# felipeagc/sycl-ray-tracer

Measured on AMD Instinct MI355X. Metric: Mrays/s, higher is better.
Workload: dtype f32

## Files before the change

### include/rt_mi355x.h

```cpp
#ifndef RT_MI355X_H
#define RT_MI355X_H

#include <stddef.h>
#include <stdint.h>

#ifdef __cplusplus
extern "C" {
#endif

#define RT_ABI_VERSION 8

typedef enum rt_status {
    RT_OK = 0,
    RT_ERR_INVALID = -1,
    RT_ERR_NO_DEVICE = -2,
    RT_ERR_HIP = -3,
    RT_ERR_OOM = -4,
    RT_ERR_UNSUPPORTED = -5
} rt_status;

#define RT_TEX_SIZE 512u
#define RT_TEX_CHANNELS 4u
#define RT_TEX_MAX_LAYERS 128u

// ... 6 lines not shown
    int32_t height;
} rt_camera;

int rt_camera_init(rt_camera* out, int32_t width, int32_t height, const float center[3],
                   const float dir[3], float focal_length);

enum { RT_MAT_NONE = 0, RT_MAT_DIFFUSE = 1, RT_MAT_METALLIC = 2, RT_MAT_DIELECTRIC = 3 };
enum { RT_TEX_COLOR = 0, RT_TEX_IMAGE = 1 };

typedef struct rt_material {
    uint32_t type;
    uint32_t tex_kind;
    float color[3];
    uint32_t tex_layer;
    float emissive[3];
    float roughness;
    float ior;
} rt_material;

typedef struct rt_instance {
    float transform[16];
    float normal_mat[9];
    uint32_t material;
} rt_instance;

typedef struct rt_scene_desc {
    uint32_t n_vertices;
    const float* positions;
    const float* normals;
    const float* uvs;
    uint32_t n_triangles;
    const uint32_t* indices;
    const uint32_t* tri_instance;
    uint32_t n_instances;
    const rt_instance* instances;
    uint32_t n_materials;
    const rt_material* materials;
    uint32_t n_layers;
    const uint8_t* textures;
    float sky[3];
} rt_scene_desc;

typedef struct rt_scene rt_scene;
typedef struct rt_renderer rt_renderer;

enum { RT_BVH_DEFAULT = 0, RT_BVH_LBVH = 1, RT_BVH_SAH = 2, RT_BVH_LBVH_GPU = 3 };

int rt_scene_create(const rt_scene_desc* desc, int device, int bvh_kind, rt_scene** out);
void rt_scene_destroy(rt_scene* scene);

#define RT_SCENE_UPDATABLE 1u
int rt_scene_create_ex(const rt_scene_desc* desc, int device, int bvh_kind, uint32_t flags, rt_scene** out);
#define RT_SCENE_KEEP_PREVIOUS 2u

typedef struct rt_scene_update_desc {
    uint32_t n_instances;
    const rt_instance* instances;
    uint32_t n_vertices;
    const float* positions;
    const float* normals;
} rt_scene_update_desc;
typedef struct rt_update_stats { double device_ms; uint32_t launches; uint32_t refit_nodes; } rt_update_stats;
int rt_scene_update(rt_scene* scene, const rt_scene_update_desc* u, rt_update_stats* stats);

typedef struct rt_scene_info_t {
    uint32_t n_triangles;
    uint32_t n_nodes;
    uint32_t max_depth;
    uint32_t max_leaf_tris;
    float bounds_lo[3];
    float bounds_hi[3];
    double sah_cost;
    uint64_t device_bytes;
    uint32_t n_leaf_records;
    uint32_t n_split_triangles;
} rt_scene_info_t;
int rt_scene_info(const rt_scene* scene, rt_scene_info_t* out);

int rt_scene_check_bvh(const rt_scene* scene);
int rt_scene_count_visits(const rt_scene* scene, uint32_t n, const float* org, const float* dir, int mode,
                          uint64_t* node_visits, uint64_t* tri_tests, float* t, uint32_t* tri);

int rt_intersect_batch(rt_scene* scene, uint32_t n, const float* org, const float* dir, float* t,
                       float* u, float* v, uint32_t* tri);

enum { RT_QUERY_CLOSEST = 0, RT_QUERY_ANY = 1 };
#define RT_TRI_REJECTED 0xFFFFFFFEu
typedef struct rt_ray_query {
    uint32_t n;
    uint32_t mode;
    const float* org;
    const float* dir;
    const float* tmax;
    float* t;
    float* u;
    float* v;
    uint32_t* tri;
    uint8_t* occluded;
} rt_ray_query;
int rt_trace_rays(rt_scene* scene, const rt_ray_query* q);
int rt_trace_rays_device(rt_scene* scene, const rt_ray_query* q, void* stream);

typedef struct rt_path_query {
    uint32_t n;
    uint32_t max_depth;
    uint32_t samples;
    uint32_t rr_start;
    const float* org;
    const float* dir;
    const uint32_t* rng;
    uint32_t* rng_out;
    float* radiance;
    uint32_t* rays;
} rt_path_query;
int rt_trace_paths(rt_scene* scene, const rt_path_query* q);
int rt_trace_paths_device(rt_scene* scene, const rt_path_query* q, void* stream);

enum {
    RT_RENDERER_MEGAKERNEL = 0,
    RT_RENDERER_WAVEFRONT = 1
};
enum { RT_SEED_DEFAULT = 0, RT_SEED_WAVEFRONT = 1, RT_SEED_MEGAKERNEL = 2 };

int rt_renderer_create(int kind, rt_scene* scene, int32_t width, int32_t height,
                       uint32_t max_depth, uint32_t sample_count, uint32_t seed_mode,
                       rt_renderer** out);
void rt_renderer_destroy(rt_renderer* r);

int rt_renderer_set_tile(rt_renderer* r, uint32_t rank, uint32_t world, uint32_t strip_rows);
int32_t rt_renderer_local_rows(const rt_renderer* r);
int32_t rt_renderer_global_row(const rt_renderer* r, int32_t local_row);

int rt_renderer_set_profiling(rt_renderer* r, int enable);

int rt_renderer_set_russian_roulette(rt_renderer* r, uint32_t start_bounce);

int rt_renderer_set_frame_seed(rt_renderer* r, uint32_t salt);

#define RT_SCHED_ALL_BOUNCES 0xFFFFFFFFu
typedef struct rt_schedule {
    uint32_t finish_depth;
    uint32_t samples_per_launch;
    uint32_t stream_lanes;
    int32_t requeue;
    uint32_t reorder;
    uint32_t matsort;
    int32_t cost_order;
    uint32_t hip_graph;
    uint32_t fused_bounce;
    int32_t pixel_slices;
} rt_schedule;
int rt_renderer_set_schedule(rt_renderer* r, const rt_schedule* s);
int rt_renderer_get_schedule(const rt_renderer* r, rt_schedule* out);

enum {
    RT_K_MEGAKERNEL = 0,
    RT_K_WF_INIT = 1,
    RT_K_WF_GENERATE = 2,
    RT_K_WF_EXTEND = 3,
    RT_K_WF_SHADE = 4,
    RT_K_WF_SHADE_REORDER = 5,
    RT_K_WF_SHADE_MATSORT = 6,
    RT_K_WF_FINISH = 7,
    RT_K_WF_FINISH_REQUEUE = 8,
    RT_K_WF_TILE_ORDER = 9,
    RT_K_WF_RESOLVE = 10,
    RT_K_FILL_BLACK = 11,
    RT_K_WF_SHOOT = 12,
    RT_K_BLOCK_RESOLVE = 13,
    RT_K_COUNT = 16
};

typedef struct rt_stats {
    uint64_t rays;
    double seconds;
    double device_ms;
    double hot_kernel_ms;
    uint32_t hot_kernel_launches;
    uint32_t launches;
    uint32_t launches_by_kernel[RT_K_COUNT];
    uint32_t stream_lanes;
    uint32_t samples_per_launch;
    uint32_t finish_depth;
    uint32_t cost_ordered;
    double kernel_ms[RT_K_COUNT];
    uint32_t hw_queues;
    uint32_t pixel_slices;
} rt_stats;

int rt_render_frame(rt_renderer* r, const rt_camera* cam, float* rgba_f32, uint8_t* rgba_u8,
                    rt_stats* stats);

int rt_render_frame_device(rt_renderer* r, const rt_camera* cam, void* d_rgba_f32,
                           void* d_rgba_u8, void* stream, rt_stats* stats);

int rt_render_frame_begin(rt_renderer* r, const rt_camera* cam, void* d_rgba_f32, void* d_rgba_u8, void* stream);
int rt_render_frame_end(rt_renderer* r, rt_stats* stats);

int rt_renderer_set_progressive(rt_renderer* r, int enable);
int rt_render_frame_continue(rt_renderer* r, uint32_t samples, float* rgba_f32, uint8_t* rgba_u8, rt_stats* stats);
int rt_render_frame_continue_device(rt_renderer* r, uint32_t samples, void* d_rgba_f32, void* d_rgba_u8,
                                    void* stream, rt_stats* stats);
int rt_renderer_accumulated_samples(const rt_renderer* r, uint32_t* out);

int rt_renderer_block_grid(const rt_renderer* r, uint32_t* blocks_x, uint32_t* blocks_y);
int rt_render_frame_continue_blocks(rt_renderer* r, uint32_t samples, const uint32_t* blocks, uint32_t n_blocks,
                                    float* rgba_f32, uint8_t* rgba_u8, rt_stats* stats);
int rt_render_frame_continue_blocks_device(rt_renderer* r, uint32_t samples, const uint32_t* blocks, uint32_t n_blocks,
                                           void* d_rgba_f32, void* d_rgba_u8, void* stream, rt_stats* stats);
int rt_renderer_block_samples(const rt_renderer* r, uint32_t* out);
int rt_renderer_adapt(rt_renderer* r, float threshold, uint32_t min_samples, uint32_t* blocks_out, uint32_t* n_out);
int rt_render_frame_continue_adaptive(rt_renderer* r, uint32_t samples, float threshold, uint32_t min_samples,
                                      float* rgba_f32, uint8_t* rgba_u8, rt_stats* stats, uint32_t* n_blocks_out);
int rt_render_frame_continue_adaptive_device(rt_renderer* r, uint32_t samples, float threshold, uint32_t min_samples,
                                             void* d_rgba_f32, void* d_rgba_u8, void* stream, rt_stats* stats,
                                             uint32_t* n_blocks_out);
int rt_renderer_block_errors(const rt_renderer* r, float* out);

int rt_scene_gbuffer(rt_scene* scene, const rt_camera* cam, float* albedo, float* normal, float* position);
int rt_scene_gbuffer_device(rt_scene* scene, const rt_camera* cam, void* d_albedo, void* d_normal, void* d_position, void* stream);

int rt_scene_gbuffer_motion(rt_scene* scene, const rt_camera* cam, float* albedo, float* normal, float* position, float* prev_position);
// ... 93 lines not shown
```

### sycl-ray-tracer_amd/csrc/rt_abi.hip

```cpp
#include "bvh_quantise.h"
#include "rt_internal.h"

namespace rtlib {
thread_local std::string g_err;

int copy_out(const rt_renderer* r, int rc, float* rgba_f32, uint8_t* rgba_u8) {
    if (rc != RT_OK) return rc;
    if (rgba_f32 && r->n_local) HIPCHK(hipMemcpy(rgba_f32, r->d_f32, (size_t)r->n_local * 16, hipMemcpyDeviceToHost));
    if (rgba_u8 && r->n_local) HIPCHK(hipMemcpy(rgba_u8, r->d_u8, (size_t)r->n_local * 4, hipMemcpyDeviceToHost));
    return RT_OK;
}
}

extern "C" {

const char* rt_last_error(void) { return g_err.c_str(); }
int rt_abi_version(void) { return RT_ABI_VERSION; }

int rt_device_count(void) {
    int n = 0;
    hipError_t e = hipGetDeviceCount(&n);
    if (e != hipSuccess) return fail(RT_ERR_NO_DEVICE, std::string("hipGetDeviceCount: ") + hipGetErrorString(e));
    return n;
}

int rt_camera_init(rt_camera* out, int32_t width, int32_t height, const float center[3], const float dir_in[3],
                   float focal_length) {
    if (!out || !center || !dir_in || width <= 0 || height <= 0) return fail(RT_ERR_INVALID, "bad camera arguments");
    auto norm = [](const float v[3], float o[3]) {
        float inv = 1.0f / std::sqrt((v[0] * v[0] + v[1] * v[1]) + v[2] * v[2]);
        o[0] = v[0] * inv, o[1] = v[1] * inv, o[2] = v[2] * inv;
    };
    auto cross = [](const float a[3], const float b[3], float o[3]) {
        o[0] = a[1] * b[2] - a[2] * b[1], o[1] = a[2] * b[0] - a[0] * b[2], o[2] = a[0] * b[1] - a[1] * b[0];
    };
    float dir[3], right[3], up[3], tmp[3];
    const float world_up[3] = {0.0f, 1.0f, 0.0f};
    norm(dir_in, dir);
    cross(dir, world_up, tmp), norm(tmp, right);
    cross(right, dir, tmp), norm(tmp, up);
    const float vp0 = 1.0f * ((float)width / (float)height), vp1 = 1.0f;
    const float du_div = (float)width / (vp0 * 2.0f), dv_div = (float)height / (vp1 * 2.0f);
    for (int a = 0; a < 3; ++a) {
        const float viewport_u = (-right[a]) * vp0, viewport_v = up[a] * vp1;
        out->center[a] = center[a];
        out->pixel00[a] = ((center[a] + viewport_u) + viewport_v) + dir[a] * focal_length;
        out->delta_u[a] = right[a] / du_div;
        out->delta_v[a] = (-up[a]) / dv_div;
    }
    out->width = width, out->height = height;
    return RT_OK;
}

int rt_scene_create(const rt_scene_desc* desc, int device, int bvh_kind, rt_scene** out) { return rt_scene_create_ex(desc, device, bvh_kind, 0u, out); }

int rt_scene_create_ex(const rt_scene_desc* desc, int device, int bvh_kind, uint32_t flags, rt_scene** out) {
    if (!out) return fail(RT_ERR_INVALID, "null output pointer");
    *out = nullptr;
    if (flags & ~(RT_SCENE_UPDATABLE | RT_SCENE_KEEP_PREVIOUS)) return fail(RT_ERR_INVALID, "unknown scene flags");
    if ((flags & RT_SCENE_KEEP_PREVIOUS) && !(flags & RT_SCENE_UPDATABLE)) return fail(RT_ERR_INVALID, "RT_SCENE_KEEP_PREVIOUS is a flag of updatable scenes: pass RT_SCENE_UPDATABLE with it");
    if (bvh_kind != RT_BVH_DEFAULT && bvh_kind != RT_BVH_LBVH && bvh_kind != RT_BVH_SAH && bvh_kind != RT_BVH_LBVH_GPU)
        return fail(RT_ERR_INVALID, "unknown bvh_kind");
    if (bvh_kind == RT_BVH_LBVH_GPU) {
        if (device < 0) return fail(RT_ERR_NO_DEVICE, "RT_BVH_LBVH_GPU needs a device (device >= 0)");
        int rc0 = device_ok(device);
        if (rc0 != RT_OK) return rc0;
    }
    rt_scene* s = new (std::nothrow) rt_scene();
    if (!s) return fail(RT_ERR_OOM, "host allocation failed");
    std::string err;
    int rc = RT_OK;
    try {
        rc = build_host_scene(desc, bvh_kind, s->hs, err);
    } catch (const std::bad_alloc&) {
        delete s;
        return fail(RT_ERR_OOM, "host allocation failed while building the scene");
    } catch (const std::exception& e) {
        delete s;
        return fail(RT_ERR_INVALID, std::string("scene build failed: ") + e.what());
    }
    if (rc != RT_OK) {
        delete s;
        return fail(rc, err);
    }
    s->device = device;
    if (device >= 0) {
        rc = device_ok(device);
        if (rc == RT_OK) {
            if (s->hs.nodes.size() > (size_t)(0x7FFFFFFF / 64)) {
                rt_scene_destroy(s);
                return fail(RT_ERR_INVALID, "BVH too large for 32-bit node offsets");
            }
            std::vector<BvhNode> dn(s->hs.nodes);
            for (BvhNode& n : dn)
                for (int k = 0; k < 4; ++k)
                    if (n.child[k] >= 0) n.child[k] *= 64;
            rc = upload(dn, &s->dev.nodes, s->device_bytes);
        }
        if (rc == RT_OK) {
            std::vector<uint8_t> packed(s->hs.tris.size() * (size_t)kTriBytes + 48, 0);
            for (size_t i = 0; i < s->hs.tris.size(); ++i) std::memcpy(packed.data() + i * kTriBytes, &s->hs.tris[i], std::min<size_t>(kTriBytes, sizeof(TriRec)));
            rc = upload(packed, &s->dev.tris, s->device_bytes);
        }
        if (rc == RT_OK) rc = upload(s->hs.shade, &s->dev.shade, s->device_bytes);
        if (rc == RT_OK) {
            std::vector<InstRec> rows(s->hs.inst);
            if (flags & RT_SCENE_UPDATABLE) rows.resize(std::max<size_t>(rows.size(), desc->n_instances));
            rc = upload(rows, &s->dev.inst, s->device_bytes);
        }
        if (rc == RT_OK) rc = upload(s->hs.mats, &s->dev.mats, s->device_bytes);
        if (rc == RT_OK) rc = upload(s->hs.tex, &s->dev.tex, s->device_bytes);
        if (rc == RT_OK && hipMalloc((void**)&s->d_query_cursor, kQueryCursorBytes) != hipSuccess)
            rc = fail(RT_ERR_OOM, "device allocation failed (the ray-query cursors)");
        if (rc != RT_OK) {
            rt_scene_destroy(s);
            return rc;
        }
        s->dev.n_nodes = (uint32_t)s->hs.nodes.size();
        s->dev.n_tris = (uint32_t)(s->hs.wverts.size() / 9);
        std::memcpy(s->dev.sky, s->hs.sky, 12);
        s->dev.packed_mat = s->hs.packed_mat ? 1u : 0u;
        const bool stage = s->hs.packed_mat && s->hs.n_layers <= 65536u;
        s->dev.lds_nm = stage ? (uint32_t)std::min<size_t>(s->hs.inst.size(), kLdsNm) : 0u;
        s->dev.lds_mats = stage ? (uint32_t)std::min<size_t>(s->hs.mats.size(), kLdsMats) : 0u;
        scene_cells(s->hs, s->dev);
    }
    if (flags & RT_SCENE_UPDATABLE) {
        rc = no_throw([&] { return init_scene_update(s, desc, (flags & RT_SCENE_KEEP_PREVIOUS) != 0); });
        if (rc != RT_OK) {
            rt_scene_destroy(s);
            return rc;
        }
    }
    *out = s;
    return RT_OK;
}

void rt_scene_destroy(rt_scene* s) {
    if (!s) return;
    if (s->device >= 0 && hipSetDevice(s->device) == hipSuccess) {
        for (auto& se : s->ev_gbuffer) (void)hipEventSynchronize(se.second), (void)hipEventDestroy(se.second);
        (void)hipFree((void*)s->dev.nodes), (void)hipFree((void*)s->dev.tris), (void)hipFree((void*)s->dev.shade);
        (void)hipFree((void*)s->dev.inst), (void)hipFree((void*)s->dev.mats), (void)hipFree((void*)s->dev.tex);
        (void)hipFree((void*)s->d_query_cursor);
    }
    free_scene_update(s);
    delete s;
}

int rt_scene_info(const rt_scene* s, rt_scene_info_t* out) {
    if (!s || !out) return fail(RT_ERR_INVALID, "null argument");
    if (const int rc = sync_host_copy(s)) return rc;
    out->n_triangles = (uint32_t)(s->hs.wverts.size() / 9);
    out->n_nodes = (uint32_t)s->hs.nodes.size();
    out->max_depth = s->hs.max_depth;
    out->max_leaf_tris = s->hs.max_leaf_tris;
    std::memcpy(out->bounds_lo, s->hs.bounds_lo, 12), std::memcpy(out->bounds_hi, s->hs.bounds_hi, 12);
    out->sah_cost = s->hs.sah_cost;
    out->device_bytes = s->device_bytes;
    out->n_leaf_records = (uint32_t)s->hs.tris.size();
    out->n_split_triangles = s->hs.n_split_triangles;
    return RT_OK;
}

int rt_scene_check_bvh(const rt_scene* s) {
    if (!s) return fail(RT_ERR_INVALID, "null scene");
    if (const int rc0 = sync_host_copy(s)) return rc0;
    std::string err;
    int rc = check_bvh(s->hs, err);
    return rc == RT_OK ? RT_OK : fail(rc, err);
}

int rt_scene_count_visits(const rt_scene* s, uint32_t n, const float* org, const float* dir, int mode, uint64_t* node_visits, uint64_t* tri_tests,
                          float* t, uint32_t* tri) {
    if (!s || (n && (!org || !dir))) return fail(RT_ERR_INVALID, "null argument");
    if (const int rc0 = sync_host_copy(s)) return rc0;
    std::string err;
    const int rc = no_throw([&] { return count_visits(s->hs, n, org, dir, mode, node_visits, tri_tests, t, tri, err); });
    return rc == RT_OK ? RT_OK : fail(rc, err.empty() ? g_err : err);
}

int rt_renderer_create(int kind, rt_scene* scene, int32_t width, int32_t height, uint32_t max_depth,
                       uint32_t sample_count, uint32_t seed_mode, rt_renderer** out) {
    if (!out) return fail(RT_ERR_INVALID, "null output pointer");
    *out = nullptr;
    if (!scene) return fail(RT_ERR_INVALID, "null scene");
    if (kind != RT_RENDERER_MEGAKERNEL && kind != RT_RENDERER_WAVEFRONT) return fail(RT_ERR_INVALID, "unknown renderer kind");
    if (width <= 0 || height <= 0 || (int64_t)width * height > (int64_t)1 << 30) return fail(RT_ERR_INVALID, "bad image size");
    if (sample_count == 0) return fail(RT_ERR_INVALID, "sample_count must be >= 1");
    if (seed_mode > RT_SEED_MEGAKERNEL) return fail(RT_ERR_INVALID, "unknown seed mode");
    if ((uint64_t)sample_count * ((uint64_t)max_depth + 1) > (1ull << 26)) return fail(RT_ERR_INVALID, "sample_count * max_depth too large");
    if (scene->device < 0) return fail(RT_ERR_NO_DEVICE, "scene was built host-only (device < 0)");
    int rc = device_ok(scene->device);
    if (rc != RT_OK) return rc;
    rt_renderer* r = new (std::nothrow) rt_renderer();
    if (!r) return fail(RT_ERR_OOM, "host allocation failed");
    r->kind = kind, r->scene = scene, r->width = width, r->height = height;
    r->scene_gen = scene->generation;
    r->max_depth = max_depth, r->spp = sample_count;
    r->seed_mode = seed_mode != RT_SEED_DEFAULT ? seed_mode
                   : (kind == RT_RENDERER_MEGAKERNEL ? RT_SEED_MEGAKERNEL : RT_SEED_WAVEFRONT);
    r->hw_queues = hw_queues_from_env();
    const char* prof = std::getenv("RT_PROFILE_KERNELS");
    r->profile_kernels = prof && prof[0] == '1';
    if (const char* e = dev_knob("RT_MEGA_LDS_PAD")) r->mega_lds_pad = (uint32_t)std::max(0, std::min(100 * 1024, std::atoi(e)));
    if (const char* e = dev_knob("RT_MEGA_OCC")) r->mega_occ = (uint32_t)std::max(1, std::min((int)kMegaWaves, std::atoi(e)));
    auto bail = [&](int code) {
        rt_renderer_destroy(r);
        return code;
    };
    {
        hipStream_t s0 = nullptr;
        bool owned = false;
        if (lane_stream_of(scene->device, 0, &s0, &owned) != hipSuccess) return bail(fail(RT_ERR_HIP, "cannot create the stream-lane pool"));
    }
    hipDeviceProp_t prop;
    if (hipGetDeviceProperties(&prop, scene->device) == hipSuccess && prop.multiProcessorCount > 0) r->n_cus = prop.multiProcessorCount;
    if (hipStreamCreateWithFlags(&r->stream, hipStreamNonBlocking) != hipSuccess) return bail(fail(RT_ERR_HIP, "hipStreamCreate failed"));
    if (hipEventCreate(&r->ev_begin) != hipSuccess || hipEventCreate(&r->ev_end) != hipSuccess ||
        hipEventCreateWithFlags(&r->ev_fork, hipEventDisableTiming) != hipSuccess || hipEventCreateWithFlags(&r->ev_tile_read, hipEventDisableTiming) != hipSuccess)
        return bail(fail(RT_ERR_HIP, "hipEventCreate failed"));
    if (hipMalloc((void**)&r->d_frame, sizeof(MegaFrame)) != hipSuccess || hipHostMalloc((void**)&r->h_frame, sizeof(MegaFrame)) != hipSuccess)
        return bail(fail(RT_ERR_OOM, "frame constant buffer allocation failed"));
// ... 284 lines not shown
```

### sycl-ray-tracer_amd/csrc/rt_device.h

```cpp
#pragma once
#include <hip/hip_runtime.h>

#include "../../include/rt_mi355x.h"
#include "rt_types.h"

namespace rt {

#define RT_DEV __device__ __forceinline__

struct f3 {
    float x, y, z;
};
RT_DEV f3 mk3(float x, float y, float z) { return f3{x, y, z}; }
RT_DEV f3 operator+(f3 a, f3 b) { return mk3(a.x + b.x, a.y + b.y, a.z + b.z); }
RT_DEV f3 operator-(f3 a, f3 b) { return mk3(a.x - b.x, a.y - b.y, a.z - b.z); }
RT_DEV f3 operator-(f3 a) { return mk3(-a.x, -a.y, -a.z); }
RT_DEV f3 operator*(f3 a, f3 b) { return mk3(a.x * b.x, a.y * b.y, a.z * b.z); }
RT_DEV f3 operator*(float s, f3 a) { return mk3(s * a.x, s * a.y, s * a.z); }
RT_DEV f3 operator*(f3 a, float s) { return mk3(a.x * s, a.y * s, a.z * s); }
RT_DEV float dot3(f3 a, f3 b) { return (a.x * b.x + a.y * b.y) + a.z * b.z; }
RT_DEV f3 cross3(f3 a, f3 b) {
    return mk3(a.y * b.z - a.z * b.y, a.z * b.x - a.x * b.z, a.x * b.y - a.y * b.x);
}
RT_DEV float rcp_rn(float x) {
// ... 222 lines not shown
    lmask nx, ny, nz;
};

RT_DEV float ub0(uint32_t w) { return (float)(w & 0xffu); }
RT_DEV float ub1(uint32_t w) { return (float)((w >> 8) & 0xffu); }
RT_DEV float ub2(uint32_t w) { return (float)((w >> 16) & 0xffu); }
RT_DEV float ub3(uint32_t w) { return (float)(w >> 24); }

struct WaveStats {
    uint32_t inner_steps = 0, inner_lanes = 0, leaf_steps = 0, leaf_lanes = 0;
    uint32_t shade_rounds = 0, shade_lanes = 0, live_lane_steps = 0, top_lanes = 0;
};
RT_DEV TravSigns trav_signs(const Trav& T) { return TravSigns{lanes(T.ix < 0.0f), lanes(T.iy < 0.0f), lanes(T.iz < 0.0f)}; }
RT_DEV void trav_inner(const SceneDev& S, Trav& T, const TravStack& stack, const TopTree& top, const TravSigns& sg) {
    const float inf = __builtin_huge_valf();
    float k0, k1, k2, k3;
    u32x4 w0, w1, w2, chw;
    if (T.cur < top.count * 64) {
        const uint32_t o = (uint32_t)T.cur >> 2;
        w0 = *(lds_u32x4*)(size_t)((uint32_t)(size_t)top.w0 + o), w1 = *(lds_u32x4*)(size_t)((uint32_t)(size_t)top.w1 + o);
        w2 = *(lds_u32x4*)(size_t)((uint32_t)(size_t)top.w2 + o), chw = *(lds_u32x4*)(size_t)((uint32_t)(size_t)top.ch + o);
    } else {
        asm volatile("global_load_dwordx4 %0, %4, %5\n\t"
                     "global_load_dwordx4 %1, %4, %5 offset:16\n\t"
                     "global_load_dwordx4 %2, %4, %5 offset:32\n\t"
                     "global_load_dwordx4 %3, %4, %5 offset:48"
                     : "=&v"(w0), "=&v"(w1), "=&v"(w2), "=&v"(chw)
                     : "v"((uint32_t)T.cur), "s"(S.nodes)
                     : "memory");
    }
    asm volatile("s_waitcnt vmcnt(1)" : "+v"(w0), "+v"(w1), "+v"(w2));
    const float ax = __uint_as_float(w0.w) * T.ix;
    const float ay = __uint_as_float(w2.z) * T.iy;
    const float az = __uint_as_float(w2.w) * T.iz;
    const float bx = __builtin_fmaf(__uint_as_float(w0.x), T.ix, T.ox);
    const float by = __builtin_fmaf(__uint_as_float(w0.y), T.iy, T.oy);
    const float bz = __builtin_fmaf(__uint_as_float(w0.z), T.iz, T.oz);
    const lmask nx = sg.nx, ny = sg.ny, nz = sg.nz;
    const uint32_t qnx = sel(nx, w1.x, w1.y), qfx = sel(nx, w1.y, w1.x);
    const uint32_t qny = sel(ny, w1.z, w1.w), qfy = sel(ny, w1.w, w1.z);
    const uint32_t qnz = sel(nz, w2.x, w2.y), qfz = sel(nz, w2.y, w2.x);
#define RT_CHILD(K, CVT)                                                                                  \
    {                                                                                                    \
        const float tn = __builtin_fmaxf(__builtin_fmaxf(__builtin_fmaf(CVT(qnx), ax, bx), __builtin_fmaf(CVT(qny), ay, by)), \
                                         __builtin_fmaxf(__builtin_fmaf(CVT(qnz), az, bz), 0.0f));       \
        const float tf = __builtin_fminf(__builtin_fminf(__builtin_fmaf(CVT(qfx), ax, bx), __builtin_fmaf(CVT(qfy), ay, by)), \
                                         __builtin_fminf(__builtin_fmaf(CVT(qfz), az, bz), T.best.t));   \
        K = sel(lanes(tn <= tf), inf, tn);                                                               \
    }
    RT_CHILD(k0, ub0)
    RT_CHILD(k1, ub1)
    RT_CHILD(k2, ub2)
    RT_CHILD(k3, ub3)
#undef RT_CHILD
#define RT_CE(KA, CA, KB, CB)                                                        \
    {                                                                               \
        const lmask sw = lanes(KB < KA);                                            \
        const float ka = sel(sw, KA, KB), kb = sel(sw, KB, KA);                     \
        const int32_t ca = sel(sw, CA, CB), cb = sel(sw, CB, CA);                   \
        KA = ka, KB = kb, CA = ca, CB = cb;                                         \
    }
    asm volatile("s_waitcnt vmcnt(0)" : "+v"(chw));
    int32_t c0 = (int32_t)chw.x, c1 = (int32_t)chw.y, c2 = (int32_t)chw.z, c3 = (int32_t)chw.w;
    RT_CE(k0, c0, k1, c1)
    RT_CE(k2, c2, k3, c3)
    RT_CE(k0, c0, k2, c2)
#undef RT_CE
    const bool descend = k0 < inf;
    if (lanes(!stack_shallow(stack, T, 3u)) == 0ull) {
        *lds_at(T.sp) = c3;
        T.sp = sel(lanes(k3 < inf), T.sp, T.sp + stack.pitch);
        *lds_at(T.sp) = c2;
        T.sp = sel(lanes(k2 < inf), T.sp, T.sp + stack.pitch);
        *lds_at(T.sp) = c1;
        T.sp = sel(lanes(k1 < inf), T.sp, T.sp + stack.pitch);
        if (descend) T.cur = c0;
        else trav_pop_lds(T, stack);
    } else {
        if (k3 < inf) stk_push(stack, T, c3);
        if (k2 < inf) stk_push(stack, T, c2);
        if (k1 < inf) stk_push(stack, T, c1);
        if (descend) T.cur = c0;
        else trav_pop(T, stack);
    }
}

template <bool BATCH>
RT_DEV void trav_leaf(const SceneDev& S, Trav& T, const TravStack& stack) {
    const uint32_t code = (uint32_t)~T.cur;
    const uint32_t first = code >> 2, rem = code & 3u;
    if (BATCH) {
        static_assert(kMaxLeafTris == 2 && kTriBytes == 40, "the whole-leaf step reads a leaf as 80 contiguous bytes");
        const uint8_t* p4 = S.tris + (size_t)first * kTriBytes;
        const float4 l0 = tri_ld4(p4), l1 = tri_ld4(p4 + 16), l2 = tri_ld4(p4 + 32), l3 = tri_ld4(p4 + 48), l4 = tri_ld4(p4 + 64);
        const bool two = rem != 0u;
        tri_test_regs(l0, l1, make_float2(l2.x, l2.y), T.o, T.d, T.best);
        if (__ballot(two) != 0ull) {
            if (two) tri_test_regs(make_float4(l2.z, l2.w, l3.x, l3.y), make_float4(l3.z, l3.w, l4.x, l4.y), make_float2(l4.z, l4.w), T.o, T.d, T.best);
        }
        if (lanes(!stack_shallow(stack, T, 0u)) == 0ull) trav_pop_lds(T, stack);
        else trav_pop(T, stack);
    } else {
        tri_test(S.tris + (size_t)first * kTriBytes, T.o, T.d, T.best);
        if (rem) T.cur = ~(int32_t)(((first + 1u) << 2) | (rem - 1u));
        else trav_pop(T, stack);
    }
}

template <bool STATS = false, bool LEAF_BATCH = false>
RT_DEV uint32_t trav_step_wave(const SceneDev& S, Trav& T, const TravStack& stack, const TopTree& top, const TravSigns& sg, WaveStats* ws = nullptr) {
    const bool inner = T.cur >= 0;
    const bool leaf = T.cur < 0 && T.cur != kTravDone;
    const uint32_t ni = (uint32_t)__popcll(__ballot(inner)), nl = (uint32_t)__popcll(__ballot(leaf));
    if (ni * 3u >= nl * 4u && !(LEAF_BATCH && nl >= 64u)) {
        if (STATS && ni) ws->inner_steps++, ws->inner_lanes += ni, ws->top_lanes += (uint32_t)__popcll(__ballot(inner && T.cur < kTopNodes * 64));
        if (inner) trav_inner(S, T, stack, top, sg);
    } else {
        if (STATS) ws->leaf_steps++, ws->leaf_lanes += (uint32_t)__popcll(__ballot(leaf));
        if (leaf) trav_leaf<LEAF_BATCH>(S, T, stack);
    }
    return ni + nl;
}

RT_DEV Hit intersect(const SceneDev& S, f3 o, f3 d, const TravStack& stack, const TopTree& top) {
    Trav T;
    trav_begin(T, o, d, stack);
    const TravSigns sg = trav_signs(T);
    while (trav_step_wave(S, T, stack, top, sg)) {}
    return T.best;
}

RT_DEV bool near_zero3(f3 e) {
    const float s = 1e-8f;
    return (__builtin_fabsf(e.x) < s) && (__builtin_fabsf(e.y) < s) && (__builtin_fabsf(e.z) < s);
}
RT_DEV float length_squared3(f3 v) {
    float l = __builtin_sqrtf(dot3(v, v));
    return l * l;
}
RT_DEV f3 reflect3(f3 v, f3 n) { return v - (2.0f * dot3(v, n)) * n; }
RT_DEV f3 refract3(f3 uv, f3 n, float etai_over_etat) {
    float cos_theta = __builtin_fminf(dot3(-uv, n), 1.0f);
    f3 r_out_perp = etai_over_etat * (uv + cos_theta * n);
    f3 r_out_parallel = (-__builtin_sqrtf(__builtin_fabsf(1.0f - length_squared3(r_out_perp)))) * n;
    return r_out_perp + r_out_parallel;
}
RT_DEV float schlick(float cosine, float ref_idx) {
    float r0 = (1.0f - ref_idx) / (1.0f + ref_idx);
    r0 = r0 * r0;
    float x = 1.0f - cosine;
    float x2 = x * x;
    float x5 = (x2 * x2) * x;
    return r0 + (1.0f - r0) * x5;
}
RT_DEV float unorm8_to_float(uint32_t b) {
    const float x = (float)b, r = 1.0f / 255.0f;
    const float q = x * r;
    return __builtin_fmaf(__builtin_fmaf(-q, 255.0f, x), r, q);
}

RT_DEV bool albedo_is_texture(const MatRec& m) { return (m.type == RT_MAT_DIFFUSE || m.type == RT_MAT_METALLIC) && m.tex_kind != RT_TEX_COLOR; }
RT_DEV uint32_t albedo_fetch(const SceneDev& S, const MatRec& m, float u, float v) {
    float fu = u - __builtin_floorf(u);
    float fv = v - __builtin_floorf(v);
    int iu = (int)__builtin_floorf(fu * 512.0f);
    int iv = (int)__builtin_floorf(fv * 512.0f);
    iu = iu < 0 ? 0 : (iu > 511 ? 511 : iu);
    iv = iv < 0 ? 0 : (iv > 511 ? 511 : iv);
    return *reinterpret_cast<const uint32_t*>(S.tex + (((size_t)m.tex_layer * 512u + (size_t)iv) * 512u + (size_t)iu) * 4u);
}
RT_DEV f3 albedo_decode(uint32_t texel) {
    return mk3(unorm8_to_float(texel & 0xffu), unorm8_to_float((texel >> 8) & 0xffu), unorm8_to_float((texel >> 16) & 0xffu));
}
RT_DEV f3 albedo(const SceneDev& S, const MatRec& m, float u, float v) {
    if (m.tex_kind == RT_TEX_COLOR) return mk3(m.color[0], m.color[1], m.color[2]);
    float fu = u - __builtin_floorf(u);
    float fv = v - __builtin_floorf(v);
    int iu = (int)__builtin_floorf(fu * 512.0f);
    int iv = (int)__builtin_floorf(fv * 512.0f);
    iu = iu < 0 ? 0 : (iu > 511 ? 511 : iu);
    iv = iv < 0 ? 0 : (iv > 511 ? 511 : iv);
    const uint32_t texel = *reinterpret_cast<const uint32_t*>(
// ... 129 lines not shown
        nm[0] = __uint_as_float(a.x), nm[1] = __uint_as_float(a.y), nm[2] = __uint_as_float(a.z), nm[3] = __uint_as_float(a.w);
        nm[4] = __uint_as_float(b.x), nm[5] = __uint_as_float(b.y), nm[6] = __uint_as_float(b.z), nm[7] = __uint_as_float(b.w);
        nm[8] = __uint_as_float(c);
    } else {
        const InstRec* inst = S.inst + (S.packed_mat ? (iw & kPackedInstMask) : iw);
        u32x4 a, b;
        uint32_t c;
        asm volatile("global_load_dwordx4 %0, %3, off\n\t"
                     "global_load_dwordx4 %1, %3, off offset:16\n\t"
                     "global_load_dword %2, %3, off offset:32\n\t"
                     "s_waitcnt vmcnt(0)"
                     : "=&v"(a), "=&v"(b), "=&v"(c)
                     : "v"(inst)
                     : "memory");
        nm[0] = __uint_as_float(a.x), nm[1] = __uint_as_float(a.y), nm[2] = __uint_as_float(a.z), nm[3] = __uint_as_float(a.w);
        nm[4] = __uint_as_float(b.x), nm[5] = __uint_as_float(b.y), nm[6] = __uint_as_float(b.z), nm[7] = __uint_as_float(b.w);
        nm[8] = __uint_as_float(c);
    }
    const f3 g = mk3((nm[0] * vn.x + nm[3] * vn.y) + nm[6] * vn.z, (nm[1] * vn.x + nm[4] * vn.y) + nm[7] * vn.z,
                     (nm[2] * vn.x + nm[5] * vn.y) + nm[8] * vn.z);
    const f3 normal = normalize3(g);
    RT_STAMP_AFTER(ck, 3, normal.x);
    f3 sdir, satt;
#ifdef RT_SCATTER_PRIO
    __builtin_amdgcn_s_setprio(RT_SCATTER_PRIO);
#endif
    const bool scattered = scatter<true>(S, mat, rng, d, normal, tu, tv, sdir, satt, texel);
    RT_STAMP_AFTER(ck, 4, satt.x);
    if (scattered) {
        org = mk3(org.x + dir.x * h.t, org.y + dir.y * h.t, org.z + dir.z * h.t);
        dir = sdir;
        att = att * satt;
        return false;
    }
    if constexpr (is_no_sink<Sink>::value) result = att * rad;
    else sink(att * rad);
    return true;
}

RT_DEV uint8_t to_unorm8(float c) { return (uint8_t)__builtin_rintf(clamp01(c) * 255.0f); }

#define RT_TRAVERSAL_LDS(BLOCK)                                                                        \
    __shared__ u32x4 top_all[4 * kTopNodes];  \
    u32x4 *const top_w0 = top_all, *const top_w1 = top_all + kTopNodes, *const top_w2 = top_all + 2 * kTopNodes, *const top_ch = top_all + 3 * kTopNodes; \
    __shared__ int32_t lds_stack[kLdsStack * (BLOCK)];                                                 \
    int32_t spill[kStackSize - kLdsStack];                                                             \
    const int32_t top_count = (int32_t)S.n_nodes < kTopNodes ? (int32_t)S.n_nodes : kTopNodes;         \
    top_tree_fill(S, top_w0, top_w1, top_w2, top_ch, top_count);                                       \
    __syncthreads();                                                                                   \
    const TopTree top{(lds_u32x4*)top_w0, (lds_u32x4*)top_w1, (lds_u32x4*)top_w2, (lds_u32x4*)top_ch, top_count}; \
    const TravStack stack{(uint32_t)(size_t)(lds_i32*)(lds_stack + threadIdx.x), spill, 4u * (BLOCK)}; \
    lds_stack[threadIdx.x] = kTravDone;

#define RT_SHADE_LDS                                                                                   \
    __shared__ u32x4 shade_nm[3 * kLdsNm], shade_mat[2 * kLdsMats];                                    \
    shade_tables_fill(S, shade_nm, shade_mat);                                                         \
    const ShadeTables tab{(lds_u32x4*)shade_nm, (lds_u32x4*)shade_mat, S.lds_nm, S.lds_mats};


}
```

### sycl-ray-tracer_amd/csrc/rt_frame.hip

```cpp
#include "rt_internal.h"
#include "rt_kernels.h"



namespace rtlib {

void drop_graph(rt_renderer* r) {
    if (r->graph_exec) (void)hipGraphExecDestroy(r->graph_exec);
    r->graph_exec = nullptr;
}

void free_block_state(rt_renderer* r) {
    if (r->d_blk) (void)hipFree(r->d_blk);
    if (r->d_snap) (void)hipFree(r->d_snap);
    if (r->h_blk) (void)hipHostFree(r->h_blk);
    r->d_blk = nullptr, r->d_snap = nullptr, r->h_blk = nullptr;
    r->blocks_x = r->blocks_y = 0;
    r->h_block_count.clear();
}
size_t blk_words(const rt_renderer* r) { return std::max<size_t>((size_t)r->blocks_x * r->blocks_y, 1); }
int alloc_block_state(rt_renderer* r) {
    free_block_state(r);
    if (!r->d_carry) return RT_OK;
    r->blocks_x = ((uint32_t)r->width + 7u) / 8u, r->blocks_y = ((uint32_t)r->tile.local_rows + 7u) / 8u;
// ... 311 lines not shown
    free_tile_buffers(r);
    r->unusable = true, r->n_local = 0, r->tile.local_rows = 0;
    g_err = msg;
    return rc;
}
int alloc_tile_buffers(rt_renderer* r) {
    const int rc = alloc_tile_buffers_impl(r);
    if (rc != RT_OK) return mark_unusable(r, rc);
    r->unusable = false;
    return RT_OK;
}

CameraDev to_dev(const rt_camera& c) {
    CameraDev d;
    std::memcpy(d.center, c.center, 12), std::memcpy(d.pixel00, c.pixel00, 12);
    std::memcpy(d.du, c.delta_u, 12), std::memcpy(d.dv, c.delta_v, 12);
    d.width = c.width, d.height = c.height;
    return d;
}

hipEvent_t pool_event(std::vector<hipEvent_t>& pool, size_t i) {
    while (pool.size() <= i) {
        hipEvent_t e;
        if (hipEventCreate(&e) != hipSuccess) return nullptr;
        pool.push_back(e);
    }
    return pool[i];
}

__global__ void __launch_bounds__(256) k_fill_words(uint32_t* __restrict__ p, uint32_t n, uint32_t v) {
    const uint32_t i = blockIdx.x * 256u + threadIdx.x;
    if (i < n) p[i] = v;
}
__global__ void __launch_bounds__(64) k_copy_words(uint32_t* __restrict__ dst, const uint32_t* __restrict__ src, uint32_t n) {
    if (threadIdx.x < n) dst[threadIdx.x] = src[threadIdx.x];
}
int fill_bytes(void* p, int byte, size_t bytes, hipStream_t st, bool capturing) {
    if (!capturing) {
        HIPCHK(hipMemsetAsync(p, byte, bytes, st));
        return RT_OK;
    }
    const uint32_t n = (uint32_t)(bytes / 4), b = (uint32_t)(byte & 0xFF);
    if (n) hipLaunchKernelGGL(k_fill_words, dim3((n + 255u) / 256u), dim3(256), 0, st, (uint32_t*)p, n, b * 0x01010101u);
    return RT_OK;
}

using FinishKernel = decltype(&k_wf_finish<false, false>);
template <bool ST>
FinishKernel finish_variant(bool shoot, bool req, bool sliced, bool carry, bool blocks) {
    if (shoot) return k_wf_finish<ST, false, true>;
    if (sliced) return blocks ? k_wf_finish<ST, false, false, true, true, true> : carry ? k_wf_finish<ST, false, false, true, true> : k_wf_finish<ST, false, false, true>;
    return req ? k_wf_finish<ST, true> : k_wf_finish<ST, false>;
}
FinishKernel finish_kernel(bool stats, bool shoot, bool req, bool sliced, bool carry, bool blocks) {
    return stats ? finish_variant<true>(shoot, req, sliced, carry, blocks) : finish_variant<false>(shoot, req, sliced, carry, blocks);
}
using MegaKernel = decltype(&k_megakernel<0, false>);
template <int ST, bool SL>
MegaKernel mega_carry(CarryMode carry) {
    switch (carry) {
    case kCarryStore: return k_megakernel<ST, SL, kCarryStore>;
    case kCarryLoadStore: return k_megakernel<ST, SL, kCarryLoadStore>;
    case kCarryBlocks: return k_megakernel<ST, SL, kCarryBlocks>;
    default: return k_megakernel<ST, SL, kCarryNone>;
    }
}
template <int ST>
MegaKernel mega_sliced(bool sliced, CarryMode carry) { return sliced ? mega_carry<ST, true>(carry) : mega_carry<ST, false>(carry); }
MegaKernel mega_kernel(int stats, bool sliced, CarryMode carry) {
    return stats == 2 ? mega_sliced<2>(sliced, carry) : stats == 1 ? mega_sliced<1>(sliced, carry) : mega_sliced<0>(sliced, carry);
}
using ShadeKernel = decltype(&k_wf_shade<false, false>);
ShadeKernel shade_kernel(bool reorder, bool matsort) {
    if (reorder) return matsort ? k_wf_shade<true, true> : k_wf_shade<true, false>;
    return matsort ? k_wf_shade<false, true> : k_wf_shade<false, false>;
}

FramePlan plan_frame(const rt_renderer* r, const FrameRequest& q) {
    FramePlan p{};
    p.req = q;
    p.chunk = q.spp;
    p.sl.n_slices = 1;
    const uint32_t D = r->max_depth;
    const bool blocks = q.carry == kCarryBlocks;
    if (r->kind == RT_RENDERER_MEGAKERNEL) {
        p.hot = D == 0 ? RT_K_FILL_BLACK : RT_K_MEGAKERNEL;
        constexpr uint32_t mega_wpb = kMegaBlock / 64;
        const uint32_t tiles_x = (uint32_t)(r->width + 7) / 8u, tiles_y = (uint32_t)(r->tile.local_rows + 7) / 8u;
        const uint32_t cap = (uint32_t)r->n_cus * 4u * r->mega_occ / mega_wpb;
        p.n_tiles = blocks ? q.n_blocks : tiles_x * tiles_y;
        p.grid = std::max<uint32_t>(1u, std::min<uint32_t>((p.n_tiles + mega_wpb - 1u) / mega_wpb, cap));
        if (const char* e = dev_knob("RT_MEGA_CHAIN_GRID_PCT"))
            p.grid = std::max<uint32_t>(1u, std::min<uint32_t>((uint32_t)((unsigned long long)p.grid * std::strtoul(e, nullptr, 10) / 100u), cap));
        p.sl = mega_slices(r, q.spp, p.n_tiles * 64u, p.grid);
        return p;
    }
    const uint32_t K = (uint32_t)r->lanes.size();
    p.lanes = K;
    p.D0 = std::min(D, r->sched.finish_depth);
    p.hot = p.D0 >= D && D > 0 ? (r->sched.fused_bounce ? RT_K_WF_SHOOT : RT_K_WF_EXTEND) : RT_K_WF_FINISH;
    for (uint32_t k = 0; k < K; ++k) {
        const uint32_t n = r->lanes[k].n_local;
        if (n) p.chunk = std::min(p.chunk, wf_chunk(r, q.spp, n));
        p.lane_pixels[k] = blocks ? 0u : n;
    }
    if (blocks) {
        const uint32_t W = (uint32_t)r->width, rows = (uint32_t)r->tile.local_rows, sr = r->tile.strip_rows;
        for (uint32_t i = 0; i < q.n_blocks; ++i) {
            const uint32_t bx = q.blocks[i] % r->blocks_x, by = q.blocks[i] / r->blocks_x, cols = std::min(8u, W - bx * 8u);
            for (uint32_t row = by * 8u; row < std::min(by * 8u + 8u, rows); ++row) p.lane_pixels[(row / sr) % K] += cols;
        }
    }
    p.requeue = wf_uses_requeue(r);
    p.spread = wf_spread(r);
    p.shoot_frame = r->sched.fused_bounce && p.D0 > 0;
    p.lpt = wf_cost_order(r, q.spp) && p.chunk == q.spp && p.D0 == 0 && D > 0 && !blocks;
    if (!p.lpt) p.sl = mega_slices(r, q.spp, p.lane_pixels[0], finish_grid(r, K, p.lane_pixels[0], q.spp > 1 && !p.requeue).grid);
    return p;
}

int next_slice_tag(rt_renderer* r, uint32_t spp, hipStream_t st, SliceDev* sl) {
    if (r->d_slice_state && r->slice_tag > 0xFFFFFFFFu - 2u * (spp + 1u)) {
// ... 107 lines not shown
                }
                hipEvent_t e0 = nullptr, e1 = nullptr, e2 = nullptr;
                if (r->profile_kernels) {
                    e0 = pool_event(L.ev_pool, ne[k]), e1 = pool_event(L.ev_pool, ne[k] + 1), e2 = pool_event(L.ev_pool, ne[k] + 2);
                    if (!e0 || !e1 || !e2) return fail(RT_ERR_HIP, "hipEventCreate failed");
                    HIPCHK(hipEventRecord(e0, ls));
                }
                hipLaunchKernelGGL(extend, dim3(ext_grid[k]), dim3(kExtendBlock), 0, ls, S, L.q[buf[k]], L.d_hits, counts + d, cursors + (size_t)s * D + d,
                                   r->d_stats);
                if (r->profile_kernels) HIPCHK(hipEventRecord(e1, ls));
                const int last = d + 1 == D ? 1 : 0, rr = r->rr_start && d + 1 >= r->rr_start && d + 1 < D ? 1 : 0;
                hipLaunchKernelGGL(shade, dim3(grid[k]), dim3(256), 0, ls, S, L.q[buf[k]], L.q[buf[k] ^ 1], L.d_hits, L.d_rng, L.d_accum, counts + d,
                                   counts + d + 1, last, rr);
                if (r->profile_kernels) {
                    HIPCHK(hipEventRecord(e2, ls));
                    L.spans.push_back({(uint32_t)ne[k], (uint32_t)ne[k] + 1, RT_K_WF_EXTEND});
                    L.spans.push_back({(uint32_t)ne[k] + 1, (uint32_t)ne[k] + 2, RT_K_WF_SHADE});
                    ne[k] += 3;
                }
                launches.add(RT_K_WF_EXTEND), launches.add(RT_K_WF_SHADE);
                if (r->sched.reorder) launches.also(RT_K_WF_SHADE_REORDER);
                if (r->sched.matsort) launches.also(RT_K_WF_SHADE_MATSORT);
                buf[k] ^= 1;
            }
        }
        if (D0 < D) {
            for (uint32_t k = 0; k < K; ++k) {
                auto& L = r->lanes[k];
                const uint32_t nq = p.lane_pixels[k];
                if (nq == 0) continue;
                hipStream_t ls = lane_stream(L);
                uint32_t* counts = L.d_counts + (size_t)s * (D + 1);
                uint32_t* cursors = L.d_counts + L.h_counts.size();
                const bool req = p.requeue && n_samples > 1;
                const FinishGrid fg = finish_grid(r, K, nq, n_samples > 1 && !req);
                hipEvent_t e0 = nullptr, e1 = nullptr;
                if (r->profile_kernels) {
                    e0 = pool_event(L.ev_pool, ne[k]), e1 = pool_event(L.ev_pool, ne[k] + 1);
                    if (!e0 || !e1) return fail(RT_ERR_HIP, "hipEventCreate failed");
                    HIPCHK(hipEventRecord(e0, ls));
                }
                unsigned long long* extra = L.d_extra + s;
                if (r->d_slice_state && !p.lpt) {
                    SliceDev sl = p.sl;
                    if (int rc_ = next_slice_tag(r, spp, ls, &sl)) return rc_;
                    r->h_frame->cam = *r->h_cam, r->h_frame->sl = sl;
                    HIPCHK(hipMemcpyAsync(r->d_frame, r->h_frame, sizeof(MegaFrame), hipMemcpyHostToDevice, ls));
                }
                FinishRequeue fq{L.d_rq_entries, L.d_rq_ctl, reinterpret_cast<uint32_t*>(L.d_extra + spp), L.rq_capacity};
                if (req) {
                    if (int rc_ = fill_bytes(L.d_rq_entries, 0xFF, (size_t)L.n_local * (n_samples - 1u) * 8, ls, capturing)) return rc_;
                    if (int rc_ = fill_bytes(L.d_rq_ctl, 0, 80 * 4, ls, capturing)) return rc_;
                }
                const FinishKernel finish = finish_kernel(r->d_stats != nullptr, false, req, p.sl.n_slices > 1u, p.req.carry >= kCarryLoadStore, blocks);
                hipLaunchKernelGGL(finish, dim3(fg.grid), dim3(kMegaBlock), 0, ls, S, r->d_cam, L.tile, L.q[buf[k]], counts + D0, cursors + (size_t)s * D + D0,
                                   L.d_rng, L.d_accum, extra, D0, D, n_samples, r->rr_start, r->d_stats, fq, fg.chunk_slots,
                                   p.lpt && s == 0 ? L.d_cost : (uint8_t*)nullptr, QueueDev{}, (uint32_t*)nullptr, 0u, p.shoot_frame ? 1u : 0u, r->d_frame,
                                   p.sl.n_slices);
                if (r->profile_kernels) {
                    HIPCHK(hipEventRecord(e1, ls));
                    L.spans.push_back({(uint32_t)ne[k], (uint32_t)ne[k] + 1, RT_K_WF_FINISH});
                    ne[k] += 2;
                }
                launches.add(RT_K_WF_FINISH);
                if (req) launches.also(RT_K_WF_FINISH_REQUEUE);
            }
        }
        s += n_samples;
    }
    HIPCHK(hipGetLastError());
    for (uint32_t k = 0; k < K; ++k) {
        auto& L = r->lanes[k];
        if (L.n_local) {
            if (blocks)
                hipLaunchKernelGGL(k_wf_resolve_blocks, dim3(grid[k]), dim3(256), 0, lane_stream(L), L.n_local, (uint32_t)r->width, r->tile.strip_rows, K, k,
                                   (const uint32_t*)r->d_blk, L.d_accum, d_f32, d_u8, (const uint32_t*)L.d_rng, (u32x4*)r->d_carry);
            else if (p.req.carry != kCarryNone)
                hipLaunchKernelGGL(k_wf_resolve<true>, dim3(grid[k]), dim3(256), 0, lane_stream(L), L.n_local, p.req.carry_total, (uint32_t)r->width,
                                   r->tile.strip_rows, K, k, L.d_accum, d_f32, d_u8, (const uint32_t*)L.d_rng, (u32x4*)r->d_carry);
            else
                hipLaunchKernelGGL(k_wf_resolve<false>, dim3(grid[k]), dim3(256), 0, lane_stream(L), L.n_local, spp, (uint32_t)r->width,
                                   r->tile.strip_rows, K, k, L.d_accum, d_f32, d_u8, (const uint32_t*)nullptr, (u32x4*)nullptr);
            launches.add(RT_K_WF_RESOLVE);
        }
        L.n_hot = ne[k];
        ne_total += ne[k];
        if (K > 1) {
            HIPCHK(hipEventRecord(L.ev_done, lane_stream(L)));
            HIPCHK(hipStreamWaitEvent(st, L.ev_done, 0));
        }
    }
    HIPCHK(hipGetLastError());
    *n_hot_events = ne_total;
    *launches_out = launches;
    return RT_OK;
}

int enqueue_frame(rt_renderer* r, const FramePlan& p, const rt_camera* cam, float* d_f32, uint8_t* d_u8, hipStream_t st, rt_stats* stats,
                  size_t* n_hot_events) {
    const CameraDev c = to_dev(*cam);
    const SceneDev& S = r->scene->dev;
    LaunchCount launches;
    *n_hot_events = 0;
    if (r->n_local == 0) {
        if (stats) stats->launches = 0, stats->pixel_slices = 1;
        return RT_OK;
    }
    const bool blocks = p.req.carry == kCarryBlocks;
    if (r->kind == RT_RENDERER_MEGAKERNEL) {
        HIPCHK(hipMemsetAsync(r->d_ray_counter, 0, 8 * sizeof(unsigned long long), st));
        hipEvent_t e0 = pool_event(r->ev_pool, 0), e1 = pool_event(r->ev_pool, 1);
        if (!e0 || !e1) return fail(RT_ERR_HIP, "hipEventCreate failed");
        SliceDev sl = p.sl;
        if (int rc_ = next_slice_tag(r, p.req.spp, st, &sl)) return rc_;
        r->h_frame->cam = c, r->h_frame->sl = sl;
        r->h_frame->carry = r->d_carry, r->h_frame->carry_total = p.req.carry_total;
        r->h_frame->n_blocks = blocks ? p.req.n_blocks : 0u;
        r->h_frame->seed_add = frame_seed_add(r);
        r->h_frame->blocks = r->d_blk ? r->d_blk + 5 * blk_words(r) + 1 : nullptr, r->h_frame->block_count = r->d_blk;
        HIPCHK(hipMemcpyAsync(r->d_frame, r->h_frame, sizeof(MegaFrame), hipMemcpyHostToDevice, st));
        if (blocks && r->max_depth > 0 && (d_f32 || d_u8)) {
            hipLaunchKernelGGL(k_blocks_resolve, dim3((r->n_local + 255u) / 256u), dim3(256), 0, st, r->n_local, (uint32_t)r->width, r->blocks_x,
                               (const u32x4*)r->d_carry, (const uint32_t*)r->d_blk, d_f32, d_u8);
            launches.add(RT_K_BLOCK_RESOLVE);
        }
        HIPCHK(hipEventRecord(e0, st));
        if (r->max_depth == 0) {
            hipLaunchKernelGGL(k_fill_black, dim3((r->n_local + 255u) / 256u), dim3(256), 0, st, r->n_local, d_f32, d_u8);
            launches.add(p.hot);
        } else if (!blocks || p.req.n_blocks) {
            if (r->d_stats) {
                HIPCHK(hipMemsetAsync(r->d_stats, 0, 13 * sizeof(unsigned long long), st));
                HIPCHK(hipMemsetAsync(r->d_stats + 13, 0xff, 2 * sizeof(unsigned long long), st));
                HIPCHK(hipMemsetAsync(r->d_stats + 15, 0, 9 * sizeof(unsigned long long), st));
            }
            const MegaKernel mega = mega_kernel(r->d_stats ? r->stats_level : 0, p.sl.n_slices > 1u, p.req.carry);
            const uint32_t pad = r->mega_lds_pad;
            if (pad) (void)hipFuncSetAttribute((const void*)mega, hipFuncAttributeMaxDynamicSharedMemorySize, (int)pad);
            hipLaunchKernelGGL(mega, dim3(p.grid), dim3(kMegaBlock), pad, st, S, r->d_frame, c.width, c.height, r->tile, r->max_depth, p.req.spp, r->seed_mode,
                               r->rr_start, d_f32, d_u8, r->d_ray_counter, r->d_stats, p.sl.n_slices);
            launches.add(p.hot);
        }
        HIPCHK(hipGetLastError());
        HIPCHK(hipEventRecord(e1, st));
        *n_hot_events = 2;
    } else {
        *r->h_cam = c;
        size_t ne_total = 0;
        if (!(r->sched.hip_graph && !r->profile_kernels && !r->d_stats)) {
            int rc = enqueue_wavefront(r, p, d_f32, d_u8, st, &launches, &ne_total);
            if (rc != RT_OK) return rc;
        } else {
            if (!r->graph_exec || r->graph_f32 != d_f32 || r->graph_u8 != d_u8 || r->graph_stream != st) {
                drop_graph(r);
                hipGraph_t g = nullptr;
                HIPCHK(hipStreamBeginCapture(st, hipStreamCaptureModeRelaxed));
                const int rc = enqueue_wavefront(r, p, d_f32, d_u8, st, &r->graph_launches, &ne_total, true);
                const hipError_t ce = hipStreamEndCapture(st, &g);
                if (rc != RT_OK || ce != hipSuccess || !g) {
                    if (g) (void)hipGraphDestroy(g);
                    return rc != RT_OK ? rc : fail(RT_ERR_HIP, std::string("hipStreamEndCapture: ") + hipGetErrorString(ce));
                }
                const hipError_t ie = hipGraphInstantiate(&r->graph_exec, g, nullptr, nullptr, 0);
                (void)hipGraphDestroy(g);
                if (ie != hipSuccess) {
                    r->graph_exec = nullptr;
                    return fail(RT_ERR_HIP, std::string("hipGraphInstantiate: ") + hipGetErrorString(ie));
                }
                r->graph_f32 = d_f32, r->graph_u8 = d_u8, r->graph_stream = st;
                r->graph_captures++;
            }
            HIPCHK(hipGraphLaunch(r->graph_exec, st));
            launches = r->graph_launches;
        }
        *n_hot_events = ne_total;
    }
    if (stats) {
        stats->stream_lanes = p.lanes;
        stats->finish_depth = p.D0;
        stats->samples_per_launch = p.chunk;
        stats->cost_ordered = launches.by[RT_K_WF_TILE_ORDER] ? 1u : 0u;
        stats->pixel_slices = p.sl.n_slices;
        stats->launches = launches.total;
        std::memcpy(stats->launches_by_kernel, launches.by, sizeof(launches.by));
    }
    return RT_OK;
}

int alloc_carry(rt_renderer* r) {
    if (r->d_carry) (void)hipFree(r->d_carry);
    r->d_carry = nullptr, r->carry_samples = 0;
    free_block_state(r);
    if (!r->progressive || r->unusable) return RT_OK;
    HIPCHK(hipMalloc(&r->d_carry, std::max<size_t>(r->n_local, 1) * 16));
// ... 325 lines not shown
```

### sycl-ray-tracer_amd/csrc/rt_internal.h

```cpp
#pragma once
#include <hip/hip_runtime.h>

#include <chrono>
#include <cmath>
#include <cstdio>
#include <cstring>
#include <map>
#include <mutex>
#include <new>
#include <string>
#include <vector>

#include "../../include/rt_mi355x.h"
#include "rt_knobs.h"
#include "rt_launch.h"
#include "scene_build.h"

namespace rtlib {

extern thread_local std::string g_err;

inline int fail(int code, const std::string& msg) {
    g_err = msg;
    return code;
// ... 40 lines not shown
    T* as() const { return static_cast<T*>(p); }
};

template <typename T>
int upload(const std::vector<T>& v, const T** out, uint64_t& bytes) {
    *out = nullptr;
    const size_t n = std::max<size_t>(v.size(), 1);
    void* p = nullptr;
    HIPCHK(hipMalloc(&p, n * sizeof(T)));
    *out = (const T*)p;
    bytes += n * sizeof(T);
    if (!v.empty()) HIPCHK(hipMemcpy(p, v.data(), v.size() * sizeof(T), hipMemcpyHostToDevice));
    return RT_OK;
}

}

using namespace rt;
using namespace rtlib;

struct SceneUpdate {
    std::vector<rt_instance> instances;
    std::vector<uint64_t> inst_use;
    std::vector<uint32_t> inst_slot;
    std::vector<uint32_t> level_nodes, level_start;
    uint32_t n_vertices = 0;
    std::vector<float> positions, normals;
    std::vector<uint32_t> indices, tri_instance;
    float* d_pos = nullptr;
    float* d_pos_stage = nullptr;
    uint32_t* d_idx = nullptr;
    uint32_t* d_tri_inst = nullptr;
    float* d_xf = nullptr;
    float* d_xf_stage = nullptr;
    uint32_t* d_islot = nullptr;
    float* d_wv = nullptr;
    float* d_wv_prev = nullptr;
    bool keep_previous = false;
    float* d_box = nullptr;
    uint32_t* d_levels = nullptr;
    unsigned long long* d_red = nullptr;
    unsigned long long* h_red = nullptr;
    hipStream_t stream = nullptr;
    hipEvent_t ev0 = nullptr, ev1 = nullptr;
    bool host_stale = false;
};

constexpr uint32_t kQueryCursorBytes = 32u * 128u;

struct rt_scene {
    HostScene hs;
    int device = -1;
    SceneDev dev{};
    uint64_t device_bytes = 0;
    SceneUpdate* upd = nullptr;
    uint64_t generation = 0;
    uint32_t frames_pending = 0;
    std::vector<std::pair<hipStream_t, hipEvent_t>> ev_gbuffer;
    unsigned long long* d_query_cursor = nullptr;
    hipStream_t query_stream = nullptr;
    bool query_launched = false;
    uint32_t query_grid[2] = {0u, 0u};
    uint32_t path_grid = 0u;
};

namespace rtlib {
inline int scene_stream_event(rt_scene* s, hipStream_t st, hipEvent_t* out) {
    for (const auto& se : s->ev_gbuffer)
        if (se.first == st) return *out = se.second, RT_OK;
    hipEvent_t ev = nullptr;
    HIPCHK(hipEventCreateWithFlags(&ev, hipEventDisableTiming));
    try {
        s->ev_gbuffer.emplace_back(st, ev);
    } catch (const std::bad_alloc&) {
        (void)hipEventDestroy(ev);
        return fail(RT_ERR_OOM, "host allocation failed");
    }
    *out = ev;
    return RT_OK;
}
}

struct LaunchCount {
    uint32_t total = 0;
    uint32_t by[RT_K_COUNT] = {};
    void add(int kernel, uint32_t n = 1) { total += n, by[kernel] += n; }
    void also(int kernel, uint32_t n = 1) { by[kernel] += n; }
};

enum CarryMode : int {
    kCarryNone = 0,
    kCarryStore = 1,
    kCarryLoadStore = 2,
    kCarryBlocks = 3,
};
struct FrameRequest {
    uint32_t spp = 0;
    CarryMode carry = kCarryNone;
    uint32_t carry_total = 0;
    const uint32_t* blocks = nullptr;
    uint32_t n_blocks = 0;
};

inline bool wants_slices(int32_t pixel_slices) { return pixel_slices != 0 && pixel_slices != 1; }

constexpr uint32_t kMaxLanes = 8;
// ... 144 lines not shown
```

### sycl-ray-tracer_amd/csrc/rt_kernels.h

```cpp
#pragma once
#include <cstddef>

#include "rt_bounce.h"
#include "rt_device.h"
#include "rt_launch.h"

namespace rt {

RT_DEV void queue_store(const QueueDev& q, uint32_t slot, uint32_t id, const RayState& r) {
    q.org_id[slot] = make_float4(r.org.x, r.org.y, r.org.z, __uint_as_float(id));
    q.a[slot] = make_uint2((uint32_t)r.dir[0] | ((uint32_t)r.dir[1] << 16), (uint32_t)r.dir[2] | ((uint32_t)r.att[0] << 16));
    q.b[slot] = make_uint2((uint32_t)r.att[1] | ((uint32_t)r.att[2] << 16), (uint32_t)r.rad[0] | ((uint32_t)r.rad[1] << 16));
    q.c[slot] = r.rad[2];
}
RT_DEV uint32_t queue_load(const QueueDev& q, uint32_t slot, RayState& r) {
    const float4 o = q.org_id[slot];
    const uint2 a = q.a[slot], b = q.b[slot];
    const uint16_t c = q.c[slot];
    r.org = mk3(o.x, o.y, o.z);
    r.dir[0] = (uint16_t)a.x, r.dir[1] = (uint16_t)(a.x >> 16), r.dir[2] = (uint16_t)a.y;
    r.att[0] = (uint16_t)(a.y >> 16), r.att[1] = (uint16_t)b.x, r.att[2] = (uint16_t)(b.x >> 16);
    r.rad[0] = (uint16_t)b.y, r.rad[1] = (uint16_t)(b.y >> 16), r.rad[2] = c;
    return __float_as_uint(o.w);
}
// ... 100 lines not shown
    cam.dv[0] = __uint_as_float(c.y), cam.dv[1] = __uint_as_float(c.z), cam.dv[2] = __uint_as_float(c.w);
    cam.width = width, cam.height = height;
    seed_add = s;
    return cam;
}
struct SliceNow {
    u32x4 head;
    u32x2 cuts;
};
RT_DEV SliceNow frame_slices(const MegaFrame* f) {
    static_assert(offsetof(SliceDev, tag0) == offsetof(SliceDev, state) + 8 && offsetof(SliceDev, shift) == offsetof(SliceDev, state) + 12, "SliceNow::head");
    SliceNow n;
    asm volatile("s_load_dwordx4 %0, %2, %3\n\t"
                 "s_load_dwordx2 %1, %2, %4\n\t"
                 "s_waitcnt lgkmcnt(0)"
                 : "=&s"(n.head), "=&s"(n.cuts)
                 : "s"(f), "i"((uint32_t)offsetof(MegaFrame, sl.state)), "i"((uint32_t)offsetof(MegaFrame, sl.cuts)));
    return n;
}
RT_DEV uint32_t frame_slice_bound(const MegaFrame* f, uint32_t j) {
    uint32_t v;
    const uint32_t at = (uint32_t)__builtin_amdgcn_readfirstlane((int)((uint32_t)offsetof(MegaFrame, sl.bound) + 4u * j));
    asm volatile("s_load_dword %0, %1, %2\n\t"
                 "s_waitcnt lgkmcnt(0)"
                 : "=&s"(v)
                 : "s"(f), "s"(at));
    return v;
}
RT_DEV u32x4* frame_carry(const MegaFrame* f) { return (u32x4*)frame_u64<offsetof(MegaFrame, carry)>(f); }
RT_DEV uint32_t frame_carry_total(const MegaFrame* f) { return frame_u32<offsetof(MegaFrame, carry_total)>(f); }
RT_DEV uint32_t frame_n_blocks(const MegaFrame* f) { return frame_u32<offsetof(MegaFrame, n_blocks)>(f); }
RT_DEV const uint32_t* frame_blocks(const MegaFrame* f) { return (const uint32_t*)frame_u64<offsetof(MegaFrame, blocks)>(f); }
RT_DEV const uint32_t* frame_block_count(const MegaFrame* f) { return (const uint32_t*)frame_u64<offsetof(MegaFrame, block_count)>(f); }
RT_DEV uint32_t frame_slice_wait_cap(const MegaFrame* f) { return frame_u32<offsetof(MegaFrame, sl.wait_cap)>(f); }
RT_DEV u32x4 carry_word(float r, float g, float b, uint32_t rng) {
    u32x4 w;
    w.x = __float_as_uint(r), w.y = __float_as_uint(g), w.z = __float_as_uint(b), w.w = rng;
    return w;
}
typedef __attribute__((address_space(3))) uint32_t lds_u32_word;
RT_DEV bool slice_wait_count(lds_u32_word* looks, const MegaFrame* f) {
    __builtin_amdgcn_s_sleep(127);
    const uint32_t n = *looks + 1u;
    *looks = n;
    return n == frame_slice_wait_cap(f) + 1u;
}
RT_DEV bool slice_wait_over(const lds_u32_word* looks, const MegaFrame* f) { return *looks > frame_slice_wait_cap(f); }
RT_DEV lds_u32_word* slice_looks_word(const void __attribute__((address_space(3))) * lane_slot, const void __attribute__((address_space(3))) * planes) {
    uint32_t a = (uint32_t)(size_t)lane_slot;
    asm volatile("" : "+v"(a));
    const uint32_t base = (uint32_t)(size_t)planes;
    return (lds_u32_word*)(size_t)(base + 3u * kMegaBlock * 4u + (((a - base) >> 6) & ~3u));
}
template <int STATS, bool SLICED, int CARRY = 0>
__global__ void __launch_bounds__(kMegaBlock, kMegaWaves) k_megakernel(SceneDev S, const MegaFrame* frame, int32_t width, int32_t height, TileDev tile,
                                                    uint32_t max_depth, uint32_t spp, uint32_t seed_mode, uint32_t rr_start, float* __restrict__ out_f32,
                                                    uint8_t* __restrict__ out_u8,
                                                    unsigned long long* __restrict__ ray_counter,
                                                    unsigned long long* __restrict__ stats_out, uint32_t n_slices) {
    WaveStats ws;
    long long t_begin = 0, t_mark = 0, t_trav = 0, t_shade = 0;
    long long ck[8] = {0, 0, 0, 0, 0, 0, 0, 0};
    if (STATS) t_begin = t_mark = (long long)__builtin_readcyclecounter();
    unsigned long long wall_begin = 0, wall_exhausted = 0;
    if (STATS >= 2) wall_begin = wall_clock64();
    const uint32_t tiles_x = (uint32_t)(width + 7) >> 3, tiles_y = (uint32_t)(tile.local_rows + 7) >> 3;
    const uint32_t n_slots = (CARRY == 3 ? frame_n_blocks(frame) : tiles_x * tiles_y) * 64u;
    const int lane = (int)(threadIdx.x & 63u);
    uint32_t* pixel_cursor = reinterpret_cast<uint32_t*>(ray_counter + 1);
    int x = 0, gy = 0;
    uint32_t pix = 0;
    uint32_t rng = 0, s = 0, depth = 0;
    unsigned long long wave_rays = 0;
    __shared__ float color_lds[3 * kMegaBlock + (SLICED ? kMegaBlock / 64 : 0)];
    typedef __attribute__((address_space(3))) float lds_f32;
    lds_f32* const color_r = (lds_f32*)color_lds + threadIdx.x;
    lds_f32* const color_g = color_r + kMegaBlock;
    lds_f32* const color_b = color_g + kMegaBlock;
    RayState r{};
    Trav T;
    if (SLICED) *slice_looks_word(color_r, (lds_f32*)color_lds) = 0u;
    RT_SHADE_LDS
    RT_TRAVERSAL_LDS(kMegaBlock)
    T.cur = kTravDone;
    constexpr uint32_t kPend = 0x40000000u;
    bool live = false;
    RefillPolicy refill;
    bool exhausted = false;
    uint32_t slice_j = 0;
    auto state_rsrc = [&](const SliceNow& n) {
        return __builtin_amdgcn_make_buffer_rsrc((void*)(((unsigned long long)n.head.y << 32) | n.head.x), 0, (int)((uint32_t)tile.local_rows * (uint32_t)width * 32u), 0x00020000);
    };
    auto take_slot = [&](uint32_t p, uint32_t first) {
        uint32_t t = p >> 6;
        if constexpr (CARRY == 3) t = frame_blocks(frame)[t];
        x = (int)((t % tiles_x) * 8u + (p & 7u));
        const int ly = (int)((t / tiles_x) * 8u + ((p >> 3) & 7u));
        gy = tile_global_row(tile, ly);
        pix = (uint32_t)ly * (uint32_t)width + (uint32_t)x;
        if (x < width && ly < tile.local_rows && gy < height) {
            s = first;
            if (!SLICED || first == 0) {
                depth = 0;
                if constexpr (CARRY >= 2) {
                    const u32x4 c = frame_carry(frame)[pix];
                    rng = c.w;
                    *color_r = __uint_as_float(c.x), *color_g = __uint_as_float(c.y), *color_b = __uint_as_float(c.z);
                    r = camera_ray(frame_camera(frame, width, height), x, gy, rng);
                } else {
                    uint32_t seed_add;
                    const CameraDev cam = frame_camera_and_seed(frame, width, height, seed_add);
                    rng = pixel_seed(x, gy, width, height, seed_mode) + seed_add;
                    *color_r = 0.0f, *color_g = 0.0f, *color_b = 0.0f;
                    r = camera_ray(cam, x, gy, rng);
                }
                trav_begin(T, r.org, ray_dir(r), stack);
            } else {
                depth = kPend;
            }
            live = true;
        }
    };
    {
        const uint32_t n_waves = gridDim.x * (kMegaBlock / 64u);
        if (n_slots <= n_waves * 64u && n_slices == 1u) {
            const uint32_t p = (uint32_t)lane * n_waves + blockIdx.x * (kMegaBlock / 64u) + (threadIdx.x >> 6);
            if (p < n_slots) take_slot(p, 0u);
            exhausted = true;
            if (STATS >= 2) wall_exhausted = wall_clock64();
        }
    }
    for (;;) {
        if (!exhausted) {
            const unsigned long long idle_m = __ballot(!live);
            const uint32_t cnt = (uint32_t)__popcll(idle_m);
            if (cnt >= refill.threshold()) {
                const uint32_t w = SLICED ? SliceCursor::claim_width(cnt, n_slots) : cnt;
                uint32_t base = 0;
                if (lane == 0) base = atomicAdd(pixel_cursor, w);
                base = (uint32_t)__builtin_amdgcn_readfirstlane((int)base);
                uint32_t first_here = 0, first_next = 0;
                if (SLICED) {
                    slice_j = SliceCursor::advance(slice_j, n_slices, base, n_slots);
                    if (slice_j) first_here = frame_slice_bound(frame, slice_j - 1u);
                    first_next = frame_slice_bound(frame, slice_j);
                }
                const uint32_t total_slots = SLICED ? n_slots * n_slices : n_slots;
                const uint32_t rank = __builtin_amdgcn_mbcnt_hi((uint32_t)(idle_m >> 32), __builtin_amdgcn_mbcnt_lo((uint32_t)idle_m, 0u));
                const uint32_t q = base + rank;
                if (!live && q < total_slots && rank < w) {
                    const SliceSlot m = SLICED ? SliceCursor::map(q, slice_j, n_slots, first_here, first_next) : SliceSlot{q, 0u};
                    take_slot(m.slot, m.first);
                }
                if (base + w >= total_slots) {
                    exhausted = true;
                    if (STATS >= 2) wall_exhausted = wall_clock64();
                }
            }
        }
        const uint32_t n_live = (uint32_t)__popcll(__ballot(live));
        if (n_live == 0) {
            if (exhausted) break;
            continue;
        }
        if (STATS) t_mark = (long long)__builtin_readcyclecounter();
        const TravSigns sg = trav_signs(T);
        const uint32_t n_rays = SLICED ? (uint32_t)__popcll(__ballot(live && depth < kPend)) : n_live;
        const uint32_t shade_at = n_rays * kMegaShadePct + (n_live - n_rays) * 100u;
        for (;;) {
            const bool waiting = live && T.cur == kTravDone;
            if ((uint32_t)__popcll(__ballot(waiting)) * 100u >= shade_at) break;
            if (STATS >= 2) ws.live_lane_steps += n_live;
            if (STATS == 1) ws.inner_steps += (uint32_t)kMegaUnroll;
            refill.stepped();
            (void)trav_step_wave<(STATS >= 2), true>(S, T, stack, top, sg, &ws);
#pragma unroll
            for (int k = 1; k < kMegaUnroll; ++k) {
                if (STATS >= 2) ws.live_lane_steps += n_live;
                (void)trav_step_wave<(STATS >= 2), true>(S, T, stack, top, sg, &ws);
            }
        }
        if (STATS) {
            ws.shade_rounds++;
            if (STATS >= 2) ws.shade_lanes += (uint32_t)__popcll(__ballot(live && T.cur == kTravDone));
            const long long now = (long long)__builtin_readcyclecounter();
            t_trav += now - t_mark, t_mark = now;
        }
        __builtin_amdgcn_s_setprio(RT_ROUND_PRIO);
#ifdef RT_ROUND_STAMPS
        if (STATS >= 2) ck[7] = (long long)__builtin_readcyclecounter();
#endif
        bool pixel_finished = false;
        {
            const unsigned long long traced = __ballot(live && T.cur == kTravDone && depth < kPend);
            wave_rays += (unsigned long long)__popcll(traced);
            if (SLICED && traced == 0ull && __ballot(live && depth < kPend) == 0ull && slice_wait_count(slice_looks_word(color_r, (lds_f32*)color_lds), frame) && lane == 0) atomicMax(ray_counter + 2, 1ull);
        }
        if (live && T.cur == kTravDone) {
            bool start = false;
            if (SLICED && depth >= kPend) {
                const SliceNow sn = frame_slices(frame);
                const auto rsrc = state_rsrc(sn);
                const uint32_t at = pix * 32u, tag = sn.head.z + s;
                const u32x4 w0 = __builtin_amdgcn_raw_buffer_load_b128(rsrc, (int)at, 0, 16 );
                const u32x4 w1 = __builtin_amdgcn_raw_buffer_load_b128(rsrc, (int)(at + 16u), 0, 16 );
                if ((w0.y == tag && w0.w == tag && w1.y == tag && w1.w == tag) || slice_wait_over(slice_looks_word(color_r, (lds_f32*)color_lds), frame)) {
                    *color_r = __uint_as_float(w0.x), *color_g = __uint_as_float(w0.z), *color_b = __uint_as_float(w1.x);
                    rng = w1.z;
                    start = true;
                }
            } else {
                f3 res;
                const auto add = [color_r, color_g, color_b](const f3& c) { *color_r = *color_r + c.x, *color_g = *color_g + c.y, *color_b = *color_b + c.z; };
                bool done;
                if (SLICED) {
                    done = shade_bounce<true>(S, rng, r, T.best, res, &T, &tab, STATS >= 2 ? ck : nullptr, add);
                } else {
                    done = shade_bounce<true>(S, rng, r, T.best, res, &T, &tab, STATS >= 2 ? ck : nullptr);
                    if (done) add(res);
                }
#ifdef RT_TAIL_PRIO
                __builtin_amdgcn_s_setprio(RT_TAIL_PRIO);
#endif
                depth++;
                bool killed = false;
                if (rr_start && !done && depth >= rr_start && depth < max_depth) killed = !roulette(rng, r);
                if (done || killed || depth == max_depth) {
                    s++;
                    bool handed = false;
                    SliceNow sn{};
                    if (SLICED) {
                        sn = frame_slices(frame);
                        const unsigned long long cuts = ((unsigned long long)sn.cuts.y << 32) | sn.cuts.x;
                        const uint32_t sh = sn.head.w;
                        handed = s < spp && (s & ((1u << sh) - 1u)) == 0u && ((cuts >> (s >> sh)) & 1ull) != 0ull;
                    }
                    if (SLICED && handed) {
                        live = false, pixel_finished = true;
                        const auto rsrc = state_rsrc(sn);
                        const uint32_t at = pix * 32u, tag = sn.head.z + s;
                        u32x4 w0, w1;
                        w0.x = __float_as_uint(*color_r), w0.y = tag, w0.z = __float_as_uint(*color_g), w0.w = tag;
                        w1.x = __float_as_uint(*color_b), w1.y = tag, w1.z = rng, w1.w = tag;
                        __builtin_amdgcn_raw_buffer_store_b128(w0, rsrc, (int)at, 0, 16 );
                        __builtin_amdgcn_raw_buffer_store_b128(w1, rsrc, (int)(at + 16u), 0, 16 );
                    } else if (s < spp) {
                        start = true;
                    } else {
                        live = false, pixel_finished = true;
                        float n;
                        if constexpr (CARRY == 3)
// ... 262 lines not shown
        if (done) {
            float4 acc = accum[id];
            acc.x = acc.x + clamp01(res.x), acc.y = acc.y + clamp01(res.y), acc.z = acc.z + clamp01(res.z);
            accum[id] = acc;
        } else {
            survive = !last_depth;
            if (rr_active && survive) survive = roulette(st, r);
        }
        rng[id] = st;
    }
    if (REORDER) {
        bins[threadIdx.x] = 0u, bins[threadIdx.x + 256u] = 0u;
        __syncthreads();
        uint32_t key = 0, rank_in_bin = 0;
        if (survive) {
            key = reorder_key(S, r);
            rank_in_bin = atomicAdd(&bins[key], 1u);
        }
        __syncthreads();
        const uint32_t b0 = bins[2u * threadIdx.x], b1 = bins[2u * threadIdx.x + 1u];
        uint32_t total = 0;
        const uint32_t off = block_scan_256(b0 + b1, wave_total, &total);
        if (threadIdx.x == 0) block_base = total ? atomicAdd(count_out, total) : 0u;
        __syncthreads();
        bins[2u * threadIdx.x] = off, bins[2u * threadIdx.x + 1u] = off + b0;
        __syncthreads();
        if (survive) queue_store(qout, block_base + bins[key] + rank_in_bin, id, r);
        return;
    }
    const unsigned long long mask = __ballot(survive);
    const uint32_t lane = threadIdx.x & 63u, wave = threadIdx.x >> 6;
    const uint32_t prefix = lane_rank(mask);
    if (lane == 0) wave_total[wave] = (uint32_t)__popcll(mask);
    __syncthreads();
    if (threadIdx.x == 0) {
        const uint32_t total = wave_total[0] + wave_total[1] + wave_total[2] + wave_total[3];
        block_base = total ? atomicAdd(count_out, total) : 0u;
    }
    __syncthreads();
    if (survive) {
        uint32_t slot = block_base + prefix;
        for (uint32_t w = 0; w < wave; ++w) slot += wave_total[w];
        queue_store(qout, slot, id, r);
    }
}

constexpr uint32_t kRqIdleCap = 1u << 26;
constexpr uint32_t kNoRay = 0xFFFFFFFFu;
constexpr uint32_t kRqEmpty = 0xFFFFFFFFu, kRqStage = 96u, kRqFlush = 32u, kRqClaim = 16u;
static_assert(kRqFlush + 64u <= kRqStage, "a whole wave of new entries must fit behind an unflushed stage");
RT_DEV unsigned long long rq_load64(const unsigned long long* p) { return __hip_atomic_load(p, __ATOMIC_RELAXED, __HIP_MEMORY_SCOPE_AGENT); }
RT_DEV void rq_store64(unsigned long long* p, unsigned long long v) { __hip_atomic_store(p, v, __ATOMIC_RELAXED, __HIP_MEMORY_SCOPE_AGENT); }

template <bool STATS, bool REQ, bool LIMIT = false, bool SLICED = false, bool CARRY = false, bool BLOCKS = false>
__global__ void __launch_bounds__(kMegaBlock, kMegaWaves) k_wf_finish(SceneDev S, const CameraDev* __restrict__ camp, TileDev tile, QueueDev qin,
                                                                    const uint32_t* __restrict__ count_in, uint32_t* __restrict__ cursor,
                                                                    uint32_t* __restrict__ rng_buf, float4* __restrict__ accum,
                                                                    unsigned long long* __restrict__ extra_rays, uint32_t first_depth, uint32_t max_depth,
                                                                    uint32_t n_samples, uint32_t rr_start,
                                                                    unsigned long long* __restrict__ stats_out, FinishRequeue fq, uint32_t chunk_slots, uint8_t* __restrict__ cost_out,
                                                                    QueueDev qout = QueueDev{}, uint32_t* __restrict__ count_out = nullptr, uint32_t bounce_limit = 0,
                                                                    uint32_t qflags = 0, const MegaFrame* slices = nullptr, uint32_t n_slices = 1) {
    static_assert(!(REQ && LIMIT), "the dynamic queue and the per-bounce hand-over are different schedules");
    static_assert(!(SLICED && (REQ || LIMIT)), "pixel slices belong to the one-launch schedule");
    static_assert(!CARRY || SLICED, "only the sliced schedule keeps a pixel's sums outside the accumulator");
    static_assert(!BLOCKS || CARRY, "a block continuation is a continuation");
    constexpr uint32_t kPend = 0x40000000u;
    const bool holes = (qflags & 1u) != 0u;
    __shared__ unsigned long long out_word;
    __shared__ uint32_t out_exited;
    if (LIMIT && threadIdx.x == 0) out_word = (unsigned long long)kOutBlock, out_exited = 0u;
    __shared__ uint32_t slot_lost;
    if (SLICED && threadIdx.x == 0) slot_lost = 0u;
    WaveStats ws;
    const uint32_t n = *count_in;
    const uint32_t lane = threadIdx.x & 63u;
    constexpr uint32_t kWavesPerBlock = kMegaBlock / 64;
    const uint32_t wave_id = blockIdx.x * kWavesPerBlock + (threadIdx.x >> 6);
    const uint32_t n_waves = gridDim.x * kWavesPerBlock;
    RT_SHADE_LDS
    RT_TRAVERSAL_LDS(kMegaBlock)
    __shared__ unsigned long long rq_stage_mem[REQ ? kWavesPerBlock * kRqStage : 1u];
    typedef __attribute__((address_space(3))) unsigned long long lds_u64_t;
    lds_u64_t* stage = (lds_u64_t*)rq_stage_mem + (threadIdx.x >> 6) * kRqStage;
    uint32_t staged = 0, stale = 0;
    uint32_t idle_polls = 0;
    const uint32_t total_entries = REQ ? n * (n_samples - 1u) : 0u;
    const auto accum_rsrc = __builtin_amdgcn_make_buffer_rsrc((void*)accum, 0, (int)(n * 16u), 0x00020000);
    __shared__ uint32_t xg_lds[SLICED ? 1u : kMegaBlock];
    typedef __attribute__((address_space(3))) uint32_t lds_u32_t;
    auto xg_word = [&]() {
        uint32_t a = stack.base;
        asm volatile("" : "+v"(a));
        return (lds_u32_t*)(size_t)(a - (uint32_t)(size_t)(lds_i32*)lds_stack + (uint32_t)(size_t)(lds_u32_t*)xg_lds);
    };
    const bool xg_packed = !SLICED && camp->width < 65536 && camp->height < 65536;
    __shared__ float sum_lds[SLICED ? 3u * kMegaBlock + kMegaBlock / 64u : 1u];
    typedef __attribute__((address_space(3))) float lds_f32_t;
    lds_f32_t* const sum_r = (lds_f32_t*)sum_lds + (SLICED ? threadIdx.x : 0u);
    lds_f32_t* const sum_g = sum_r + (SLICED ? kMegaBlock : 0u);
    lds_f32_t* const sum_b = sum_g + (SLICED ? kMegaBlock : 0u);
    if (SLICED) *slice_looks_word(sum_r, (lds_f32_t*)sum_lds) = 0u;
    bool chunk_dq = false;
    bool drained = false;
    bool waiting = false;
    Trav T;
    T.cur = kTravDone;
    bool live = false;
    RefillPolicy refill;
    RayState r{};
    uint32_t id = 0, rng = 0, depth = 0;
    unsigned long long wave_rays = 0;
    uint32_t samples_left = 0;
    bool first_counted = false;
    const bool tail_guided = LIMIT && (chunk_slots >> 31) != 0u;
    const uint32_t static_pct = (chunk_slots >> 16) & 0x7Fu;
    chunk_slots &= 0xFFFFu;
    uint32_t first_slots = chunk_slots;
    if (SLICED) first_slots = 0;
    if (tail_guided) {
        const uint32_t per_wave = (uint32_t)(((unsigned long long)n * static_pct / 100u) / (n_waves ? n_waves : 1u));
        first_slots = per_wave < 64u ? 64u : (per_wave & ~63u);
    }
    uint32_t seen = n_waves * first_slots;
    const uint32_t inv_waves = tail_guided ? 0x10000u / (n_waves ? n_waves : 1u) + 1u : 0u;
    const uint32_t n_total = SLICED ? n * n_slices : n;
    uint32_t slice_j = 0;
    uint32_t chunk_pos = wave_id * first_slots;
    uint32_t chunk_end = chunk_pos + first_slots < n_total ? chunk_pos + first_slots : n_total;
    bool exhausted = chunk_pos >= n_total;
    auto state_rsrc = [&](const SliceNow& sn) {
        const uint32_t n_state = BLOCKS ? (uint32_t)tile.local_rows * (uint32_t)camp->width : n;
        return __builtin_amdgcn_make_buffer_rsrc((void*)(((unsigned long long)sn.head.y << 32) | sn.head.x), 0, (int)(n_state * 32u), 0x00020000);
    };
    auto leave = [&]() {
        if (!LIMIT) return;
        uint32_t order = 0;
        if (lane == 0) order = atomicAdd(&out_exited, 1u);
        order = (uint32_t)__builtin_amdgcn_readfirstlane((int)order);
        if (order + 1u != kWavesPerBlock) return;
        const unsigned long long w = out_word;
        const uint32_t used = (uint32_t)w, base = (uint32_t)(w >> 32);
        for (uint32_t i = used + lane; i < kOutBlock; i += 64u) qout.org_id[base + i] = make_float4(0.0f, 0.0f, 0.0f, __uint_as_float(kNoRay));
    };
    if (exhausted) {
        if (!REQ) {
            leave();
            return;
        }
        chunk_pos = chunk_end = 0;
    }
    auto flush = [&]() {
        uint32_t t = 0;
        if (lane == 0) t = atomicAdd(fq.ctl + 0, staged);
        t = (uint32_t)__builtin_amdgcn_readfirstlane((int)t);
        asm volatile("s_waitcnt vmcnt(0)" ::: "memory");
        for (uint32_t i = lane; i < staged; i += 64u)
            if (t + i < fq.capacity) rq_store64(fq.entries + t + i, stage[i]);
        if (lane == 0 && t + staged > fq.capacity) __hip_atomic_store(fq.error, 2u, __ATOMIC_RELAXED, __HIP_MEMORY_SCOPE_AGENT);
        staged = 0;
// ... 77 lines not shown
                                    live = true;
                                } else if (!(holes && id == kNoRay)) {
                                    rng = rng_buf[id];
                                    depth = first_depth;
                                    samples_left = n_samples, first_counted = !holes;
                                    if (SLICED && CARRY) {
                                        const float4 a = accum[id];
                                        *sum_r = a.x, *sum_g = a.y, *sum_b = a.z;
                                    } else if (SLICED) {
                                        *sum_r = 0.0f, *sum_g = 0.0f, *sum_b = 0.0f;
                                    }
                                    if (!REQ && n_samples > 1u && xg_packed) {
                                        const uint32_t w = (uint32_t)camp->width;
                                        *xg_word() = (id % w) | ((uint32_t)tile_global_row(tile, (int)(id / w)) << 16);
                                    }
                                    trav_begin(T, r.org, ray_dir(r), stack);
                                    live = true;
                                }
                            }
                        }
                    }
                    chunk_pos += take;
                }
            }
        }
        const unsigned long long wait_m = REQ ? __ballot(waiting) : 0ull;
        if (REQ && waiting) {
            const unsigned long long e64 = rq_load64(fq.entries + id);
            samples_left = (uint32_t)e64, rng = (uint32_t)(e64 >> 32);
        }
        const uint32_t n_live = (uint32_t)__popcll(__ballot(live));
        if (n_live == 0) {
            if (!REQ) {
                if (exhausted) break;
                continue;
            }
            if (staged) flush();
            if (wait_m != 0ull) {
                if (++idle_polls > kRqIdleCap) {
                    if (lane == 0) __hip_atomic_store(fq.error, 1u, __ATOMIC_RELAXED, __HIP_MEMORY_SCOPE_AGENT);
                    break;
                }
                __builtin_amdgcn_s_sleep(8);
                continue;
            }
            if (drained) break;
            continue;
        }
        idle_polls = 0;
        const TravSigns sg = trav_signs(T);
        const uint32_t n_rays = SLICED ? (uint32_t)__popcll(__ballot(live && depth < kPend)) : n_live;
        const uint32_t shade_at = n_rays * kMegaShadePct + (n_live - n_rays) * 100u;
        for (;;) {
            const bool done_trav = live && T.cur == kTravDone;
            if ((uint32_t)__popcll(__ballot(done_trav)) * 100u >= shade_at) break;
            if (STATS) ws.live_lane_steps += n_live * kMegaUnroll;
            refill.stepped();
            (void)trav_step_wave<STATS, true>(S, T, stack, top, sg, &ws);
#pragma unroll
            for (int k = 1; k < kMegaUnroll; ++k) (void)trav_step_wave<STATS, true>(S, T, stack, top, sg, &ws);
        }
        if (STATS) ws.shade_rounds++, ws.shade_lanes += (uint32_t)__popcll(__ballot(live && T.cur == kTravDone));
        __builtin_amdgcn_s_setprio(0);
        bool requeue = false, slot_finished = false, hand_on = false;
        {
            const unsigned long long traced = __ballot(live && T.cur == kTravDone && !(SLICED && depth >= kPend));
            wave_rays += (unsigned long long)__popcll(__ballot(live && T.cur == kTravDone && !(first_counted && depth == first_depth) && !(SLICED && depth >= kPend)));
            if (SLICED && traced == 0ull && __ballot(live && depth < kPend) == 0ull && slice_wait_count(slice_looks_word(sum_r, (lds_f32_t*)sum_lds), slices) && lane == 0 && fq.error)
                __hip_atomic_store(fq.error, 4u, __ATOMIC_RELAXED, __HIP_MEMORY_SCOPE_AGENT);
        }
        if (SLICED && live && T.cur == kTravDone && depth >= kPend) {
            const SliceNow sn = frame_slices(slices);
            const auto rsrc = state_rsrc(sn);
            const uint32_t at = id * 32u, tag = sn.head.z + (n_samples - samples_left);
            const u32x4 w0 = __builtin_amdgcn_raw_buffer_load_b128(rsrc, (int)at, 0, 16 );
            const u32x4 w1 = __builtin_amdgcn_raw_buffer_load_b128(rsrc, (int)(at + 16u), 0, 16 );
            if ((w0.y == tag && w0.w == tag && w1.y == tag && w1.w == tag) || slice_wait_over(slice_looks_word(sum_r, (lds_f32_t*)sum_lds), slices)) {
                *sum_r = __uint_as_float(w0.x), *sum_g = __uint_as_float(w0.z), *sum_b = __uint_as_float(w1.x);
                rng = w1.z;
                const CameraDev cam = *camp;
                int x, gy;
                if (xg_packed) {
                    const uint32_t xg = *xg_word();
                    x = (int)(xg & 0xFFFFu), gy = (int)(xg >> 16);
                } else {
                    x = (int)(id % (uint32_t)cam.width), gy = tile_global_row(tile, (int)(id / (uint32_t)cam.width));
                }
                r = camera_ray(cam, x, gy, rng);
                depth = 0;
                trav_begin(T, r.org, ray_dir(r), stack);
            }
        } else if (live && T.cur == kTravDone) {
            f3 res;
            const bool done = shade_bounce<true>(S, rng, r, T.best, res, &T, &tab);
            depth++;
            bool ends = done;
            if (SLICED && done) {
                *sum_r = *sum_r + clamp01(res.x), *sum_g = *sum_g + clamp01(res.y), *sum_b = *sum_b + clamp01(res.z);
            } else if (done) {
                float4 acc;
                if (REQ) {
                    const u32x4 a = __builtin_amdgcn_raw_buffer_load_b128(accum_rsrc, (int)(id * 16u), 0, 16 );
                    acc = make_float4(__uint_as_float(a.x), __uint_as_float(a.y), __uint_as_float(a.z), __uint_as_float(a.w));
                } else {
                    acc = accum[id];
                }
                acc.x = acc.x + clamp01(res.x), acc.y = acc.y + clamp01(res.y), acc.z = acc.z + clamp01(res.z);
                if (REQ) {
                    u32x4 a;
                    a.x = __float_as_uint(acc.x), a.y = __float_as_uint(acc.y), a.z = __float_as_uint(acc.z), a.w = __float_as_uint(acc.w);
                    __builtin_amdgcn_raw_buffer_store_b128(a, accum_rsrc, (int)(id * 16u), 0, 16 );
                } else {
                    accum[id] = acc;
                }
            } else if (depth == max_depth) {
                ends = true;
            } else if (rr_start && depth >= rr_start) {
                ends = !roulette(rng, r);
            }
            bool handed = false;
            if (SLICED && ends && samples_left > 1u) {
                const SliceNow sn = frame_slices(slices);
                const unsigned long long cuts = ((unsigned long long)sn.cuts.y << 32) | sn.cuts.x;
                const uint32_t sh = sn.head.w, s_next = n_samples - (samples_left - 1u);
                handed = (s_next & ((1u << sh) - 1u)) == 0u && ((cuts >> (s_next >> sh)) & 1ull) != 0ull;
                if (handed) {
                    const auto rsrc = state_rsrc(sn);
                    const uint32_t at = id * 32u, tag = sn.head.z + s_next;
                    u32x4 w0, w1;
                    w0.x = __float_as_uint(*sum_r), w0.y = tag, w0.z = __float_as_uint(*sum_g), w0.w = tag;
                    w1.x = __float_as_uint(*sum_b), w1.y = tag, w1.z = rng, w1.w = tag;
                    __builtin_amdgcn_raw_buffer_store_b128(w0, rsrc, (int)at, 0, 16 );
                    __builtin_amdgcn_raw_buffer_store_b128(w1, rsrc, (int)(at + 16u), 0, 16 );
                }
            }
            if (!REQ && ends && !handed && --samples_left) {
                const CameraDev cam = *camp;
                int x, gy;
                if (xg_packed) {
                    const uint32_t xg = *xg_word();
                    x = (int)(xg & 0xFFFFu), gy = (int)(xg >> 16);
                } else {
                    x = (int)(id % (uint32_t)cam.width), gy = tile_global_row(tile, (int)(id / (uint32_t)cam.width));
                }
                r = camera_ray(cam, x, gy, rng);
// ... 213 lines not shown
```

### sycl-ray-tracer_amd/csrc/rt_types.h

```cpp
#pragma once
#include <cstdint>

namespace rt {

#ifdef __HIPCC__
#define RT_HD __host__ __device__ inline
#else
#define RT_HD inline
#endif
struct alignas(64) BvhNode {
    float origin[3];
    float scale_x;
    uint32_t q[6];
    float scale_y, scale_z;
    int32_t child[4];
    RT_HD float scale(int a) const { const float s = a == 0 ? scale_x : (a == 1 ? scale_y : scale_z); return s < 0.0f ? -s : s; }
    RT_HD void set_scale(int a, float s) { (a == 0 ? scale_x : (a == 1 ? scale_y : scale_z)) = s; }
};
static_assert(sizeof(BvhNode) == 64, "BvhNode must be 64 bytes");
constexpr int32_t kChildEmpty = (int32_t)0x80000000;
struct Box3 {
    float lo[3], hi[3];
};

RT_HD void clear_planes(BvhNode& n) {
    n.scale_x = n.scale_y = n.scale_z = 1.0f;
    n.origin[0] = n.origin[1] = n.origin[2] = 0.0f;
    for (int i = 0; i < 6; ++i) n.q[i] = (i & 1) ? 0u : 0xFFFFFFFFu;
}
RT_HD BvhNode empty_node() {
    BvhNode n;
    clear_planes(n);
    for (int k = 0; k < 4; ++k) n.child[k] = kChildEmpty;
    return n;
}
struct LeafRange {
    uint32_t first, count;
};
RT_HD LeafRange leaf_range(int32_t child) {
    const uint32_t code = (uint32_t)~child;
    return {code >> 2, (code & 3u) + 1u};
}
RT_HD int32_t leaf_child(uint32_t first, uint32_t count) { return ~(int32_t)((first << 2) | (count - 1)); }
RT_HD float child_plane(const BvhNode& n, int k, int a, int side) { return n.origin[a] + (float)((n.q[2 * a + side] >> (8 * k)) & 0xffu) * n.scale(a); }
RT_HD Box3 child_box(const BvhNode& n, int k) {
    Box3 b;
    for (int a = 0; a < 3; ++a) b.lo[a] = child_plane(n, k, a, 0), b.hi[a] = child_plane(n, k, a, 1);
    return b;
}

constexpr int kMaxLeafTris = 2;
constexpr int kTopNodes = 341;
constexpr int kStackSize = 64;
constexpr uint32_t kNoTri = 0xFFFFFFFFu;
constexpr float kTNear = 0.0001f;

struct ContractRange {
    float lo[3], hi[3];
    float limit;
    uint32_t finite_only;
};
RT_HD float contract_max(float a, float b) { return a < b ? b : a; }
RT_HD bool in_contract_range(const ContractRange& r, float ox, float oy, float oz) {
    if (r.finite_only) return __builtin_isfinite(ox) && __builtin_isfinite(oy) && __builtin_isfinite(oz);
    const float o[3] = {ox, oy, oz};
    for (int a = 0; a < 3; ++a) {
        const float outside = contract_max(contract_max(r.lo[a] - o[a], o[a] - r.hi[a]), 0.0f);
        if (!(outside <= r.limit)) return false;
    }
    return true;
}

struct alignas(16) TriRec {
    float v0[3];
    float e1[3];
    float e2[3];
    uint32_t global_index;
    uint32_t pad[2];
};
static_assert(sizeof(TriRec) == 48, "TriRec must be 48 bytes");
constexpr uint32_t kTriBytes = 40;

constexpr uint32_t kPackedInstBits = 20, kPackedInstMask = (1u << kPackedInstBits) - 1u;
struct alignas(64) ShadeRec {
    float n0[3], n1[3], n2[3];
    float uv0[2], uv1[2], uv2[2];
    uint32_t instance;
};
static_assert(sizeof(ShadeRec) == 64, "ShadeRec must be 64 bytes");

constexpr uint32_t kLdsNm = 8, kLdsMats = 24;
struct alignas(16) InstRec {
    float normal_mat[9];
    uint32_t material;
    uint32_t pad[2];
};
static_assert(sizeof(InstRec) == 48, "InstRec must be 48 bytes");

struct alignas(16) MatRec {
    uint32_t type;
    uint32_t tex_kind;
    float color[3];
    uint32_t tex_layer;
    float emissive[3];
    float roughness;
    float ior;
    uint32_t pad;
};
// ... 29 lines not shown
```

### sycl-ray-tracer_amd/csrc/scene_build.cpp

```cpp
#include "scene_build.h"
#include "bvh_quantise.h"
#include "rt_knobs.h"

#include <algorithm>
#include <array>
#include <cmath>
#include <cstdio>
#include <cstdlib>
#include <cstring>
#include <limits>
#include <map>
#include <memory>
#include <deque>
#include <queue>

namespace rt {
namespace {

struct GNode {
    float lo[3], hi[3];
    int32_t left = -1, right = -1;
    uint32_t first = 0, count = 0;
    uint32_t depth = 0;
};
// ... 705 lines not shown
    }
}

void flatten(const rt_scene_desc& d, const std::vector<uint32_t>& inst_slot, HostScene& hs, std::vector<TriRec>& gtris) {
    const uint32_t T = d.n_triangles;
    world_vertices(T, d.indices, d.tri_instance, d.instances, d.positions, hs.wverts);
    hs.shade.resize(T);
    gtris.assign(T, TriRec{});
    for (uint32_t t = 0; t < T; ++t) {
        const float* p = &hs.wverts[9 * (size_t)t];
        TriRec& tr = gtris[t];
        for (int a = 0; a < 3; ++a) {
            tr.v0[a] = p[a];
            tr.e1[a] = p[3 + a] - p[a];
            tr.e2[a] = p[6 + a] - p[a];
        }
        tr.global_index = t;
        ShadeRec& s = hs.shade[t];
        const uint32_t ii = d.tri_instance[t], i0 = d.indices[3 * t], i1 = d.indices[3 * t + 1], i2 = d.indices[3 * t + 2];
        std::memcpy(s.n0, d.normals + 3 * i0, 12), std::memcpy(s.n1, d.normals + 3 * i1, 12);
        std::memcpy(s.n2, d.normals + 3 * i2, 12);
        std::memcpy(s.uv0, d.uvs + 2 * i0, 8), std::memcpy(s.uv1, d.uvs + 2 * i1, 8);
        std::memcpy(s.uv2, d.uvs + 2 * i2, 8);
        s.instance = hs.packed_mat ? (inst_slot[ii] | (d.instances[ii].material << kPackedInstBits)) : ii;
    }
}

}

int build_host_scene(const rt_scene_desc* d, int bvh_kind, HostScene& hs, std::string& err) {
    if (const int rc = validate_desc(d, bvh_kind, err)) return rc;
    hs = HostScene{};
    std::vector<uint32_t> inst_slot;
    fill_tables(*d, hs, inst_slot);
    std::vector<TriRec> gtris;
    flatten(*d, inst_slot, hs, gtris);
    if (gtris.empty()) {
        hs.built_by = (int8_t)bvh_kind;
        hs.nodes.assign(1, empty_node());
        hs.tris.assign(1, TriRec{});
        hs.tris[0].global_index = kNoTri;
        return RT_OK;
    }
    if (!world_bounds(hs.wverts, hs.bounds_lo, hs.bounds_hi, hs.pad, err)) return RT_ERR_INVALID;
    const BuildOptions options;
    for (int kind = bvh_kind;; kind = RT_BVH_MEDIAN_INTERNAL) {
        const int rc = build_tree(kind, gtris, options, hs, err);
        if (rc != kTooDeep) return rc;
        if (kind == RT_BVH_MEDIAN_INTERNAL) { err = "internal: BVH deeper than the traversal stack"; return RT_ERR_INVALID; }
        err.clear();
    }
}

void world_vertices(uint32_t n_tris, const uint32_t* indices, const uint32_t* tri_instance, const rt_instance* inst, const float* positions,
                    std::vector<float>& wv) {
    wv.resize(9 * (size_t)n_tris);
    for (uint32_t t = 0; t < n_tris; ++t) {
        const float* m = inst[tri_instance[t]].transform;
        for (int k = 0; k < 3; ++k) {
            const uint32_t vi = indices[3 * (size_t)t + k];
            const float x = positions[3 * (size_t)vi], y = positions[3 * (size_t)vi + 1], z = positions[3 * (size_t)vi + 2];
            float* p = &wv[9 * (size_t)t + 3 * k];
            p[0] = ((m[0] * x + m[4] * y) + m[8] * z) + m[12];
            p[1] = ((m[1] * x + m[5] * y) + m[9] * z) + m[13];
            p[2] = ((m[2] * x + m[6] * y) + m[10] * z) + m[14];
        }
    }
}

bool world_bounds(const std::vector<float>& wv, float lo[3], float hi[3], float& pad, std::string& err) {
    for (float v : wv)
        if (!std::isfinite(v)) { err = "non-finite world-space vertex"; return false; }
    for (int a = 0; a < 3; ++a) lo[a] = INFINITY, hi[a] = -INFINITY;
    for (size_t i = 0; i < wv.size(); ++i) {
        const int a = (int)(i % 3);
        lo[a] = std::min(lo[a], wv[i]), hi[a] = std::max(hi[a], wv[i]);
    }
    return scene_padding(lo, hi, pad, err);
}

void scene_cells(const HostScene& hs, SceneDev& dev) {
    for (int a = 0; a < 3; ++a) {
        const float ext = hs.bounds_hi[a] - hs.bounds_lo[a];
        dev.cell_lo[a] = hs.bounds_lo[a];
        dev.cell_scale[a] = ext > 0.0f && std::isfinite(ext) ? 4.0f / ext : 0.0f;
    }
}

void shading_rows(const rt_instance* inst, uint32_t n, const std::vector<uint64_t>& use, bool packed, std::vector<InstRec>& out,
                  std::vector<uint32_t>& slot) {
    slot.assign(n, 0);
    if (packed) {
        std::map<std::array<uint32_t, 9>, uint32_t> seen;
        std::vector<std::array<uint32_t, 9>> rows;
        std::vector<uint64_t> row_use;
        for (uint32_t i = 0; i < n; ++i) {
            std::array<uint32_t, 9> key;
            std::memcpy(key.data(), inst[i].normal_mat, 36);
            auto it = seen.find(key);
            if (it == seen.end()) {
                it = seen.emplace(key, (uint32_t)rows.size()).first;
                rows.push_back(key), row_use.push_back(0);
            }
            slot[i] = it->second;
            row_use[it->second] += use[i];
        }
// ... 116 lines not shown
```

### sycl-ray-tracer_amd/csrc/scene_build.h

```cpp
#pragma once
#include <cstdint>
#include <string>
#include <vector>

#include "../../include/rt_mi355x.h"
#include "rt_types.h"

namespace rt {

struct HostScene {
    std::vector<BvhNode> nodes;
    std::vector<TriRec> tris;
    std::vector<ShadeRec> shade;
    std::vector<InstRec> inst;
    std::vector<MatRec> mats;
    std::vector<uint8_t> tex;
    std::vector<float> wverts;
    std::vector<float> rec_lo, rec_hi;
    uint32_t n_split_triangles = 0;
    uint32_t n_layers = 0;
    bool packed_mat = false;
    int8_t built_by = -1;
    float sky[3] = {0.5f, 0.7f, 1.0f};
    float bounds_lo[3] = {0, 0, 0}, bounds_hi[3] = {0, 0, 0};
    float pad = 0.0f;
    uint32_t max_depth = 0, max_leaf_tris = 0, stack_need = 0;
    double sah_cost = 0.0;
};

constexpr int RT_BVH_MEDIAN_INTERNAL = 99;

int build_host_scene(const rt_scene_desc* desc, int bvh_kind, HostScene& out, std::string& err);

int build_lbvh_gpu(HostScene& hs, const std::vector<TriRec>& gtris, std::string& err);

void world_vertices(uint32_t n_tris, const uint32_t* indices, const uint32_t* tri_instance, const rt_instance* inst, const float* positions,
                    std::vector<float>& wv);
bool world_bounds(const std::vector<float>& wv, float lo[3], float hi[3], float& pad, std::string& err);
void scene_cells(const HostScene& hs, SceneDev& dev);
void record_boxes(HostScene& hs);
Box3 leaf_bounds(const HostScene& hs, int32_t child);
inline float half_area(const float* lo, const float* hi) {
    float dx = hi[0] - lo[0], dy = hi[1] - lo[1], dz = hi[2] - lo[2];
    if (!(dx >= 0 && dy >= 0 && dz >= 0)) return 0.0f;
    return dx * dy + dy * dz + dz * dx;
}

void shading_rows(const rt_instance* inst, uint32_t n, const std::vector<uint64_t>& use, bool packed, std::vector<InstRec>& rows,
                  std::vector<uint32_t>& slot);
bool scene_padding(const float lo[3], const float hi[3], float& pad, std::string& err);
void node_levels(const std::vector<BvhNode>& nodes, std::vector<uint32_t>& level_nodes, std::vector<uint32_t>& level_start);
bool refit_host(HostScene& hs, const std::vector<uint32_t>& level_nodes, std::vector<float>& box, std::string& err);
double refit_sah_cost(const HostScene& hs, const std::vector<float>& box);
double decoded_sah_cost(const HostScene& hs);

int check_bvh(const HostScene& hs, std::string& err);

int count_visits(const HostScene& hs, uint32_t n, const float* org, const float* dir, int mode, uint64_t* node_visits, uint64_t* tri_tests, float* t_out,
                 uint32_t* tri_out, std::string& err);

}
```

### sycl-ray-tracer_amd/csrc/scene_check.cpp

```cpp
#include "scene_build.h"

#include <algorithm>
#include <cmath>
#include <limits>

namespace rt {
namespace {

void grow(Box3& r, const Box3& c) {
    for (int a = 0; a < 3; ++a) r.lo[a] = std::min(r.lo[a], c.lo[a]), r.hi[a] = std::max(r.hi[a], c.hi[a]);
}

template <class Enter, class Visit>
bool exact_boxes(const HostScene& hs, int32_t child, uint32_t depth, Box3& r, Enter&& enter, Visit&& visit) {
    const float inf = std::numeric_limits<float>::infinity();
    r = Box3{{inf, inf, inf}, {-inf, -inf, -inf}};
    if (!enter(child, depth)) return false;
    if (child < 0) {
        r = leaf_bounds(hs, child);
        return true;
    }
    const BvhNode& n = hs.nodes[(size_t)child];
    for (int k = 0; k < 4; ++k) {
        if (n.child[k] == kChildEmpty) continue;
        Box3 c;
        if (!exact_boxes(hs, n.child[k], depth + 1, c, enter, visit) || !visit(child, k, c)) return false;
        grow(r, c);
    }
    return true;
}

}

double decoded_sah_cost(const HostScene& hs) {
    double cost = 0.0, root_area = 0.0;
    for (size_t i = 0; i < hs.nodes.size(); ++i) {
        const BvhNode& n = hs.nodes[i];
        Box3 nb{{INFINITY, INFINITY, INFINITY}, {-INFINITY, -INFINITY, -INFINITY}};
        for (int k = 0; k < 4; ++k) {
            if (n.child[k] == kChildEmpty) continue;
            const Box3 b = child_box(n, k);
            grow(nb, b);
            const double w = n.child[k] >= 0 ? 1.0 : (double)leaf_range(n.child[k]).count;
            cost += w * (double)half_area(b.lo, b.hi);
        }
        if (i == 0) root_area = (double)half_area(nb.lo, nb.hi);
    }
    return root_area > 0.0 ? 1.0 + cost / root_area : 0.0;
}

double refit_sah_cost(const HostScene& hs, const std::vector<float>& box) {
    if (hs.built_by == RT_BVH_LBVH_GPU) return decoded_sah_cost(hs);
    if (hs.nodes.empty() || box.size() < 6 * hs.nodes.size()) return 0.0;
    const double root_area = std::max(1e-30, (double)half_area(&box[0], &box[3]));
    double cost = 0.0;
    for (const BvhNode& n : hs.nodes)
// ... 24 lines not shown
            if (++visited > hs.nodes.size()) return fail("cycle in node graph");
            return true;
        }
        const LeafRange leaf = leaf_range(child);
        if ((size_t)leaf.first + leaf.count > hs.tris.size()) return fail("leaf range out of bounds");
        for (uint32_t k = 0; k < leaf.count; ++k) {
            const TriRec& tr = hs.tris[leaf.first + k];
            if (tr.global_index >= T) return fail("leaf triangle has bad global index");
            for (uint32_t j = 0; j < k; ++j)
                if (hs.tris[leaf.first + j].global_index == tr.global_index) return fail("triangle twice in one leaf");
            if (seen[tr.global_index]++ && !split) return fail("triangle appears in two leaves");
            const float* w = &hs.wverts[9 * (size_t)tr.global_index];
            if (tr.v0[0] != w[0] || tr.v0[1] != w[1] || tr.v0[2] != w[2]) return fail("leaf triangle data mismatch");
            if (split) pieces[tr.global_index].push_back(leaf.first + k);
        }
        return true;
    };
    auto contained = [&](int32_t node, int k, const Box3& c) {
        const Box3 d = child_box(hs.nodes[(size_t)node], k);
        for (int a = 0; a < 3; ++a)
            if (!(d.lo[a] <= c.lo[a] - 0.5f * hs.pad) || !(d.hi[a] >= c.hi[a] + 0.5f * hs.pad))
                return fail("decoded child box does not contain its subtree (node " + std::to_string(node) + ")");
        return true;
    };
    Box3 all;
    if (!exact_boxes(hs, 0, 0, all, enter, contained)) return RT_ERR_INVALID;
    for (size_t t = 0; t < T; ++t)
        if (!seen[t]) { err = "triangle " + std::to_string(t) + " is in no leaf"; return RT_ERR_INVALID; }
    if (split) {
        for (size_t t = 0; t < T; ++t) {
            if (pieces[t].size() < 2) continue;
            const float* w = &hs.wverts[9 * t];
            for (int i = 0; i <= 8; ++i)
                for (int j = 0; i + j <= 8; ++j) {
                    const double u = i / 8.0, v = j / 8.0, ww = 1.0 - u - v;
                    double p[3];
                    for (int a = 0; a < 3; ++a) p[a] = ww * w[a] + u * w[3 + a] + v * w[6 + a];
                    bool in = false;
                    for (uint32_t rec : pieces[t]) {
                        bool inside = true;
                        for (int a = 0; a < 3; ++a) {
                            const double tol = 1e-6 * (std::fabs(p[a]) + 1.0);
                            inside = inside && p[a] >= (double)hs.rec_lo[3 * (size_t)rec + a] - tol && p[a] <= (double)hs.rec_hi[3 * (size_t)rec + a] + tol;
                        }
                        in = in || inside;
                    }
                    if (!in) { err = "the pieces of split triangle " + std::to_string(t) + " do not cover it"; return RT_ERR_INVALID; }
                }
        }
    }
    return RT_OK;
}

int count_visits(const HostScene& hs, uint32_t n, const float* org, const float* dir, int mode, uint64_t* node_visits, uint64_t* tri_tests, float* t_out,
                 uint32_t* tri_out, std::string& err) {
    if (mode < 0 || mode > 2) { err = "mode: 0 quantised, 1 exact, 2 quantised with two more bits"; return RT_ERR_INVALID; }
    if (hs.nodes.empty()) { err = "no tree"; return RT_ERR_INVALID; }
    const float inf = std::numeric_limits<float>::infinity();
    std::vector<Box3> box(hs.nodes.size() * 4);
    auto tested = [&](int32_t node, int k, const Box3& c) {
        const BvhNode& nd = hs.nodes[(size_t)node];
        Box3& out = box[(size_t)node * 4 + k];
        if (mode == 0) out = child_box(nd, k);
        else for (int a = 0; a < 3; ++a) {
            if (mode == 1) {
                out.lo[a] = c.lo[a] - hs.pad, out.hi[a] = c.hi[a] + hs.pad;
            } else {
                const float q = nd.scale(a) * 0.25f;
                out.lo[a] = nd.origin[a] + std::floor((c.lo[a] - hs.pad - nd.origin[a]) / q) * q;
                out.hi[a] = nd.origin[a] + std::ceil((c.hi[a] + hs.pad - nd.origin[a]) / q) * q;
            }
        }
        return true;
    };
    Box3 all;
    (void)exact_boxes(hs, 0, 0, all, [](int32_t, uint32_t) { return true; }, tested);
    uint64_t visits = 0, tests = 0;
    for (uint32_t i = 0; i < n; ++i) {
        const float o[3] = {org[3 * i], org[3 * i + 1], org[3 * i + 2]}, d[3] = {dir[3 * i], dir[3 * i + 1], dir[3 * i + 2]};
        float inv[3];
        for (int a = 0; a < 3; ++a) inv[a] = 1.0f / (std::fabs(d[a]) < 1e-30f ? std::copysign(1e-30f, d[a]) : d[a]);
        float best = inf;
        uint32_t best_tri = kNoTri;
        int32_t stack[kStackSize * 4];
        int sp = 0;
        int32_t cur = 0;
        for (;;) {
            if (cur >= 0) {
                visits++;
                const BvhNode& nd = hs.nodes[(size_t)cur];
                float key[4];
                int32_t ch[4];
                int m = 0;
                for (int k = 0; k < 4; ++k) {
                    if (nd.child[k] == kChildEmpty) continue;
                    const Box3& b = box[(size_t)cur * 4 + k];
                    float tn = 0.0f, tf = best;
                    for (int a = 0; a < 3; ++a) {
                        const float t0 = (b.lo[a] - o[a]) * inv[a], t1 = (b.hi[a] - o[a]) * inv[a];
                        tn = std::max(tn, std::min(t0, t1)), tf = std::min(tf, std::max(t0, t1));
                    }
                    if (tn <= tf) key[m] = tn, ch[m] = nd.child[k], m++;
                }
                for (int a = 1; a < m; ++a)
                    for (int b = a; b > 0 && key[b] < key[b - 1]; --b) std::swap(key[b], key[b - 1]), std::swap(ch[b], ch[b - 1]);
                for (int a = m - 1; a >= 1; --a) stack[sp++] = ch[a];
                if (m) { cur = ch[0]; continue; }
            } else {
                const LeafRange leaf = leaf_range(cur);
                for (uint32_t k = 0; k < leaf.count; ++k) {
// ... 28 lines not shown
```

### sycl-ray-tracer_amd/rtamd/abi.py

```python
from __future__ import annotations

import ctypes as C
import os
from pathlib import Path

PKG_DIR = Path(__file__).resolve().parent.parent
REPO_DIR = PKG_DIR.parent
LIB_PATH = PKG_DIR / "csrc" / "build" / "librt_mi355x.so"

RT_OK = 0
RT_ERR_INVALID, RT_ERR_NO_DEVICE, RT_ERR_HIP, RT_ERR_OOM, RT_ERR_UNSUPPORTED = -1, -2, -3, -4, -5

RT_MAT_NONE, RT_MAT_DIFFUSE, RT_MAT_METALLIC, RT_MAT_DIELECTRIC = 0, 1, 2, 3
RT_TEX_COLOR, RT_TEX_IMAGE = 0, 1
RT_RENDERER_MEGAKERNEL, RT_RENDERER_WAVEFRONT = 0, 1
RT_SEED_DEFAULT, RT_SEED_WAVEFRONT, RT_SEED_MEGAKERNEL = 0, 1, 2
RT_BVH_DEFAULT, RT_BVH_LBVH, RT_BVH_SAH, RT_BVH_LBVH_GPU = 0, 1, 2, 3
RT_BVH_MEDIAN_INTERNAL = 99
RT_SCENE_UPDATABLE = 1
RT_SCENE_KEEP_PREVIOUS = 2
RT_TEX_SIZE = 512
RT_TEX_MAX_LAYERS = 128


class rt_camera(C.Structure):
    _fields_ = [
        ("center", C.c_float * 3),
        ("pixel00", C.c_float * 3),
        ("delta_u", C.c_float * 3),
        ("delta_v", C.c_float * 3),
        ("width", C.c_int32),
        ("height", C.c_int32),
    ]


class rt_material(C.Structure):
    _fields_ = [
        ("type", C.c_uint32),
        ("tex_kind", C.c_uint32),
        ("color", C.c_float * 3),
        ("tex_layer", C.c_uint32),
        ("emissive", C.c_float * 3),
        ("roughness", C.c_float),
        ("ior", C.c_float),
    ]


class rt_instance(C.Structure):
    _fields_ = [
        ("transform", C.c_float * 16),
        ("normal_mat", C.c_float * 9),
        ("material", C.c_uint32),
    ]


class rt_scene_desc(C.Structure):
    _fields_ = [
        ("n_vertices", C.c_uint32),
        ("positions", C.POINTER(C.c_float)),
        ("normals", C.POINTER(C.c_float)),
        ("uvs", C.POINTER(C.c_float)),
        ("n_triangles", C.c_uint32),
        ("indices", C.POINTER(C.c_uint32)),
        ("tri_instance", C.POINTER(C.c_uint32)),
        ("n_instances", C.c_uint32),
        ("instances", C.POINTER(rt_instance)),
        ("n_materials", C.c_uint32),
        ("materials", C.POINTER(rt_material)),
        ("n_layers", C.c_uint32),
        ("textures", C.POINTER(C.c_uint8)),
        ("sky", C.c_float * 3),
    ]


class rt_scene_info_t(C.Structure):
    _fields_ = [
        ("n_triangles", C.c_uint32),
        ("n_nodes", C.c_uint32),
        ("max_depth", C.c_uint32),
        ("max_leaf_tris", C.c_uint32),
        ("bounds_lo", C.c_float * 3),
        ("bounds_hi", C.c_float * 3),
        ("sah_cost", C.c_double),
        ("device_bytes", C.c_uint64),
        ("n_leaf_records", C.c_uint32),
        ("n_split_triangles", C.c_uint32),
    ]


class rt_scene_update_desc(C.Structure):
    _fields_ = [
        ("n_instances", C.c_uint32),
        ("instances", C.POINTER(rt_instance)),
        ("n_vertices", C.c_uint32),
        ("positions", C.POINTER(C.c_float)),
        ("normals", C.POINTER(C.c_float)),
    ]


class rt_update_stats(C.Structure):
    _fields_ = [
        ("device_ms", C.c_double),
        ("launches", C.c_uint32),
        ("refit_nodes", C.c_uint32),
    ]


RT_SCHED_ALL_BOUNCES = 0xFFFFFFFF
KERNELS = {"megakernel": 0, "wf_init": 1, "wf_generate": 2, "wf_extend": 3, "wf_shade": 4, "wf_shade_reorder": 5, "wf_shade_matsort": 6,
           "wf_finish": 7, "wf_finish_requeue": 8, "wf_tile_order": 9, "wf_resolve": 10, "fill_black": 11, "wf_shoot": 12,
           "block_resolve": 13}
RT_K_COUNT = 16


class rt_schedule(C.Structure):
    _fields_ = [
        ("finish_depth", C.c_uint32),
        ("samples_per_launch", C.c_uint32),
        ("stream_lanes", C.c_uint32),
        ("requeue", C.c_int32),
        ("reorder", C.c_uint32),
        ("matsort", C.c_uint32),
        ("cost_order", C.c_int32),
        ("hip_graph", C.c_uint32),
        ("fused_bounce", C.c_uint32),
        ("pixel_slices", C.c_int32),
    ]


class rt_stats(C.Structure):
    _fields_ = [
        ("rays", C.c_uint64),
        ("seconds", C.c_double),
        ("device_ms", C.c_double),
        ("hot_kernel_ms", C.c_double),
        ("hot_kernel_launches", C.c_uint32),
        ("launches", C.c_uint32),
        ("launches_by_kernel", C.c_uint32 * RT_K_COUNT),
        ("stream_lanes", C.c_uint32),
        ("samples_per_launch", C.c_uint32),
        ("finish_depth", C.c_uint32),
        ("cost_ordered", C.c_uint32),
        ("kernel_ms", C.c_double * RT_K_COUNT),
        ("hw_queues", C.c_uint32),
        ("pixel_slices", C.c_uint32),
    ]


class rt_denoise_params(C.Structure):
    _fields_ = [
        ("iterations", C.c_uint32),
        ("sigma_color", C.c_float),
        ("sigma_normal", C.c_float),
        ("sigma_position", C.c_float),
        ("sigma_albedo", C.c_float),
    ]


class rt_temporal_params(C.Structure):
    _fields_ = [
        ("max_history", C.c_uint32),
        ("sigma_position", C.c_float),
        ("cos_normal", C.c_float),
    ]
# ... 14 lines not shown
RT_TEMPORAL_MOMENTS = 1
RT_QUERY_CLOSEST, RT_QUERY_ANY = 0, 1
RT_TRI_REJECTED = 0xFFFFFFFE


class rt_ray_query(C.Structure):
    _fields_ = [
        ("n", C.c_uint32),
        ("mode", C.c_uint32),
        ("org", C.c_void_p),
        ("dir", C.c_void_p),
        ("tmax", C.c_void_p),
        ("t", C.c_void_p),
        ("u", C.c_void_p),
        ("v", C.c_void_p),
        ("tri", C.c_void_p),
        ("occluded", C.c_void_p),
    ]


class rt_path_query(C.Structure):
    _fields_ = [
        ("n", C.c_uint32),
        ("max_depth", C.c_uint32),
        ("samples", C.c_uint32),
        ("rr_start", C.c_uint32),
        ("org", C.c_void_p),
        ("dir", C.c_void_p),
        ("rng", C.c_void_p),
        ("rng_out", C.c_void_p),
        ("radiance", C.c_void_p),
        ("rays", C.c_void_p),
    ]


assert C.sizeof(rt_ray_query) == 72
assert C.sizeof(rt_path_query) == 64
assert C.sizeof(rt_denoise_params) == 20
assert C.sizeof(rt_temporal_params) == 12
assert C.sizeof(rt_denoise_var_params) == 24
assert C.sizeof(rt_material) == 44
assert C.sizeof(rt_instance) == 104
assert C.sizeof(rt_camera) == 56

_P = C.POINTER
PROTOTYPES = {
    "rt_camera_init": (C.c_int, [_P(rt_camera), C.c_int32, C.c_int32, _P(C.c_float), _P(C.c_float), C.c_float]),
    "rt_scene_create": (C.c_int, [_P(rt_scene_desc), C.c_int, C.c_int, _P(C.c_void_p)]),
    "rt_scene_destroy": (None, [C.c_void_p]),
    "rt_scene_create_ex": (C.c_int, [_P(rt_scene_desc), C.c_int, C.c_int, C.c_uint32, _P(C.c_void_p)]),
    "rt_scene_update": (C.c_int, [C.c_void_p, _P(rt_scene_update_desc), _P(rt_update_stats)]),
    "rt_scene_info": (C.c_int, [C.c_void_p, _P(rt_scene_info_t)]),
    "rt_scene_check_bvh": (C.c_int, [C.c_void_p]),
    "rt_scene_count_visits": (C.c_int, [C.c_void_p, C.c_uint32, _P(C.c_float), _P(C.c_float), C.c_int, _P(C.c_uint64), _P(C.c_uint64),
                                         _P(C.c_float), _P(C.c_uint32)]),
    "rt_intersect_batch": (C.c_int, [C.c_void_p, C.c_uint32, _P(C.c_float), _P(C.c_float), _P(C.c_float),
                                     _P(C.c_float), _P(C.c_float), _P(C.c_uint32)]),
    "rt_trace_rays": (C.c_int, [C.c_void_p, _P(rt_ray_query)]),
    "rt_trace_rays_device": (C.c_int, [C.c_void_p, _P(rt_ray_query), C.c_void_p]),
    "rt_trace_paths": (C.c_int, [C.c_void_p, _P(rt_path_query)]),
    "rt_trace_paths_device": (C.c_int, [C.c_void_p, _P(rt_path_query), C.c_void_p]),
    "rt_renderer_create": (C.c_int, [C.c_int, C.c_void_p, C.c_int32, C.c_int32, C.c_uint32, C.c_uint32,
                                     C.c_uint32, _P(C.c_void_p)]),
    "rt_renderer_destroy": (None, [C.c_void_p]),
    "rt_renderer_set_tile": (C.c_int, [C.c_void_p, C.c_uint32, C.c_uint32, C.c_uint32]),
    "rt_renderer_local_rows": (C.c_int32, [C.c_void_p]),
    "rt_renderer_global_row": (C.c_int32, [C.c_void_p, C.c_int32]),
    "rt_renderer_set_profiling": (C.c_int, [C.c_void_p, C.c_int]),
    "rt_renderer_set_russian_roulette": (C.c_int, [C.c_void_p, C.c_uint32]),
    "rt_renderer_set_frame_seed": (C.c_int, [C.c_void_p, C.c_uint32]),
    "rt_renderer_set_schedule": (C.c_int, [C.c_void_p, _P(rt_schedule)]),
    "rt_renderer_get_schedule": (C.c_int, [C.c_void_p, _P(rt_schedule)]),
    "rt_render_frame_begin": (C.c_int, [C.c_void_p, C.POINTER(rt_camera), C.c_void_p, C.c_void_p, C.c_void_p]),
    "rt_render_frame_end": (C.c_int, [C.c_void_p, C.POINTER(rt_stats)]),
    "rt_render_frame": (C.c_int, [C.c_void_p, _P(rt_camera), _P(C.c_float), _P(C.c_uint8), _P(rt_stats)]),
    "rt_render_frame_device": (C.c_int, [C.c_void_p, _P(rt_camera), C.c_void_p, C.c_void_p, C.c_void_p,
                                         _P(rt_stats)]),
    "rt_renderer_set_progressive": (C.c_int, [C.c_void_p, C.c_int]),
    "rt_render_frame_continue": (C.c_int, [C.c_void_p, C.c_uint32, _P(C.c_float), _P(C.c_uint8), _P(rt_stats)]),
    "rt_render_frame_continue_device": (C.c_int, [C.c_void_p, C.c_uint32, C.c_void_p, C.c_void_p, C.c_void_p, _P(rt_stats)]),
    "rt_renderer_accumulated_samples": (C.c_int, [C.c_void_p, _P(C.c_uint32)]),
    "rt_renderer_block_grid": (C.c_int, [C.c_void_p, _P(C.c_uint32), _P(C.c_uint32)]),
    "rt_render_frame_continue_blocks": (C.c_int, [C.c_void_p, C.c_uint32, _P(C.c_uint32), C.c_uint32, _P(C.c_float), _P(C.c_uint8), _P(rt_stats)]),
    "rt_render_frame_continue_blocks_device": (C.c_int, [C.c_void_p, C.c_uint32, _P(C.c_uint32), C.c_uint32, C.c_void_p, C.c_void_p, C.c_void_p,
                                                         _P(rt_stats)]),
    "rt_renderer_block_samples": (C.c_int, [C.c_void_p, _P(C.c_uint32)]),
    "rt_renderer_adapt": (C.c_int, [C.c_void_p, C.c_float, C.c_uint32, _P(C.c_uint32), _P(C.c_uint32)]),
    "rt_render_frame_continue_adaptive": (C.c_int, [C.c_void_p, C.c_uint32, C.c_float, C.c_uint32, _P(C.c_float), _P(C.c_uint8), _P(rt_stats),
                                                    _P(C.c_uint32)]),
    "rt_render_frame_continue_adaptive_device": (C.c_int, [C.c_void_p, C.c_uint32, C.c_float, C.c_uint32, C.c_void_p, C.c_void_p, C.c_void_p,
                                                           _P(rt_stats), _P(C.c_uint32)]),
    "rt_renderer_block_errors": (C.c_int, [C.c_void_p, _P(C.c_float)]),
    "rt_scene_gbuffer": (C.c_int, [C.c_void_p, _P(rt_camera), _P(C.c_float), _P(C.c_float), _P(C.c_float)]),
    "rt_scene_gbuffer_device": (C.c_int, [C.c_void_p, _P(rt_camera), C.c_void_p, C.c_void_p, C.c_void_p, C.c_void_p]),
    "rt_scene_gbuffer_motion": (C.c_int, [C.c_void_p, _P(rt_camera), _P(C.c_float), _P(C.c_float), _P(C.c_float), _P(C.c_float)]),
    "rt_scene_gbuffer_motion_device": (C.c_int, [C.c_void_p, _P(rt_camera), C.c_void_p, C.c_void_p, C.c_void_p, C.c_void_p, C.c_void_p]),
    "rt_temporal_create": (C.c_int, [C.c_int, C.c_int32, C.c_int32, _P(C.c_void_p)]),
    "rt_temporal_destroy": (None, [C.c_void_p]),
    "rt_temporal_reset": (C.c_int, [C.c_void_p]),
    "rt_temporal_accumulate": (C.c_int, [C.c_void_p, _P(rt_temporal_params), _P(rt_camera), _P(C.c_float), _P(C.c_float), _P(C.c_float),
                                         _P(C.c_float), _P(C.c_float), _P(C.c_uint8), _P(C.c_float)]),
    "rt_temporal_accumulate_device": (C.c_int, [C.c_void_p, _P(rt_temporal_params), _P(rt_camera), C.c_void_p, C.c_void_p, C.c_void_p, C.c_void_p,
                                                C.c_void_p, C.c_void_p, C.c_void_p, C.c_void_p]),
    "rt_temporal_create_ex": (C.c_int, [C.c_int, C.c_int32, C.c_int32, C.c_uint32, _P(C.c_void_p)]),
    "rt_temporal_accumulate_moments": (C.c_int, [C.c_void_p, _P(rt_temporal_params), _P(rt_camera), _P(C.c_float), _P(C.c_float), _P(C.c_float),
                                                 _P(C.c_float), _P(C.c_float), _P(C.c_uint8), _P(C.c_float), _P(C.c_float)]),
# ... 118 lines not shown
```

### sycl-ray-tracer_amd/rtamd/renderer.py

```python
from __future__ import annotations

import ctypes as C
from dataclasses import dataclass

import numpy as np

from . import abi
from .scenes import SceneDesc


class Camera:

    def __init__(self, img_size, center, direction, focal_length: float):
        self.c = abi.rt_camera()
        lib = abi.load_library()
        ce = (C.c_float * 3)(*[float(v) for v in center])
        di = (C.c_float * 3)(*[float(v) for v in direction])
        abi.check(lib.rt_camera_init(C.byref(self.c), int(img_size[0]), int(img_size[1]), ce, di, float(focal_length)))

    @classmethod
    def for_scene(cls, desc: SceneDesc, img_size):
        p = desc.camera
        return cls(img_size, p.position, p.direction, p.focal_length)


class Scene:

    def __init__(self, desc: SceneDesc, device: int = 0, bvh: int = abi.RT_BVH_DEFAULT, lib=None, updatable: bool = False,
                 keep_previous: bool = False):
        self.desc = desc
        self.device = device
        self._lib = lib or abi.load_library()
        self._c = desc.to_c()
        self.h = C.c_void_p()
        if updatable or keep_previous:
            flags = (abi.RT_SCENE_UPDATABLE if updatable else 0) | (abi.RT_SCENE_KEEP_PREVIOUS if keep_previous else 0)
            abi.check(self._lib.rt_scene_create_ex(C.byref(self._c), device, bvh, flags, C.byref(self.h)), self._lib)
        else:
            abi.check(self._lib.rt_scene_create(C.byref(self._c), device, bvh, C.byref(self.h)), self._lib)

    def update(self, instances=None, positions=None, normals=None) -> abi.rt_update_stats:
        u = abi.rt_scene_update_desc()
        keep = []
        if instances is not None:
            xf, nm = instances
            n = int(np.asarray(xf).shape[0])
            insts = (abi.rt_instance * max(n, 1))()
            words = np.frombuffer(insts, np.float32).reshape(-1, 26)
            words[:n, :16] = np.asarray(xf, np.float32).reshape(n, 16)
            words[:n, 16:25] = np.asarray(nm, np.float32).reshape(n, 9)
            words.view(np.uint32)[:n, 25] = np.asarray(self.desc.inst_material, np.uint32)[:n]
            u.n_instances, u.instances = n, insts
            keep.append(insts)
        if positions is not None or normals is not None:
            u.n_vertices = int(self.desc.positions.shape[0])
            for name, a in (("positions", positions), ("normals", normals)):
                if a is not None:
                    a = np.ascontiguousarray(a, np.float32).reshape(-1, 3)
                    u.n_vertices = a.shape[0]
                    setattr(u, name, abi.fptr(a))
                    keep.append(a)
        st = abi.rt_update_stats()
        abi.check(self._lib.rt_scene_update(self.h, C.byref(u), C.byref(st)), self._lib)
        self.desc = self.desc.updated(instances, positions, normals)
        return st

    def info(self) -> abi.rt_scene_info_t:
        out = abi.rt_scene_info_t()
        abi.check(self._lib.rt_scene_info(self.h, C.byref(out)), self._lib)
        return out

    def check_bvh(self) -> None:
        abi.check(self._lib.rt_scene_check_bvh(self.h), self._lib)

    def intersect(self, org: np.ndarray, dirs: np.ndarray):
        org = np.ascontiguousarray(org, np.float32).reshape(-1, 3)
        dirs = np.ascontiguousarray(dirs, np.float32).reshape(-1, 3)
        n = org.shape[0]
        t, u, v = (np.zeros(n, np.float32) for _ in range(3))
        tri = np.zeros(n, np.uint32)
        abi.check(self._lib.rt_intersect_batch(self.h, n, abi.fptr(org), abi.fptr(dirs), abi.fptr(t), abi.fptr(u),
                                               abi.fptr(v), abi.u32ptr(tri)), self._lib)
        return t, u, v, tri

    def trace(self, org: np.ndarray, dirs: np.ndarray, tmax=None, any_hit: bool = False):
        org = np.ascontiguousarray(org, np.float32).reshape(-1, 3)
        dirs = np.ascontiguousarray(dirs, np.float32).reshape(-1, 3)
        n = org.shape[0]
        if dirs.shape[0] != n:
            raise ValueError("org and dirs must hold the same number of rays")
        q = abi.rt_ray_query(n=n, mode=abi.RT_QUERY_ANY if any_hit else abi.RT_QUERY_CLOSEST, org=org.ctypes.data, dir=dirs.ctypes.data)
        if tmax is not None:
            tmax = np.ascontiguousarray(tmax, np.float32).reshape(-1)
            if tmax.shape[0] != n:
                raise ValueError("tmax must hold one value per ray")
            q.tmax = tmax.ctypes.data
        if any_hit:
            occ = np.zeros(n, np.uint8)
            q.occluded = occ.ctypes.data
            abi.check(self._lib.rt_trace_rays(self.h, C.byref(q)), self._lib)
            return occ
        t, u, v = (np.zeros(n, np.float32) for _ in range(3))
        tri = np.zeros(n, np.uint32)
        q.t, q.u, q.v, q.tri = t.ctypes.data, u.ctypes.data, v.ctypes.data, tri.ctypes.data
        abi.check(self._lib.rt_trace_rays(self.h, C.byref(q)), self._lib)
        return t, u, v, tri

    def trace_device(self, n: int, d_org: int, d_dir: int, d_tmax: int = 0, d_t: int = 0, d_u: int = 0, d_v: int = 0, d_tri: int = 0,
                     d_occluded: int = 0, any_hit: bool = False, stream: int = 0) -> None:
        q = abi.rt_ray_query(n=int(n), mode=abi.RT_QUERY_ANY if any_hit else abi.RT_QUERY_CLOSEST, org=d_org or None, dir=d_dir or None,
                             tmax=d_tmax or None, t=d_t or None, u=d_u or None, v=d_v or None, tri=d_tri or None,
                             occluded=d_occluded or None)
        abi.check(self._lib.rt_trace_rays_device(self.h, C.byref(q), C.c_void_p(stream or None)), self._lib)

    def trace_paths(self, org: np.ndarray, dirs: np.ndarray, rng: np.ndarray, max_depth: int, samples: int = 1, rr_start: int = 0) -> dict:
        org, dirs, rng = np.asarray(org), np.asarray(dirs), np.asarray(rng)
        if org.ndim != 2 or org.shape[1] != 3 or dirs.shape != org.shape:
            raise ValueError("org and dirs must both be (n, 3)")
        n = org.shape[0]
        if rng.shape != (n,):
            raise ValueError("rng must hold one state per ray, shape (n,)")
        if rng.dtype.kind not in "ui":
            raise ValueError("rng must be an integer array (xorshift32 states)")
        org = np.ascontiguousarray(org, np.float32)
# ... 580 lines not shown
```

Measured before the change: 9825.

## Add compact interleaved BVH layout with byte-offset children and inline leaves

Static scenes now get a compact BVH buffer on the host, with nodes and leaf triangle records interleaved and children encoded as byte offsets whose low bits tag leaf counts. The buffer is uploaded and used by new traversal paths in the megakernel and the wavefront finish kernel when stats, carry and requeue are off. The top of the buffer is staged raw into LDS. The inner step uses SDWA byte-extract instructions and split waitcnts to decode quantised boxes. The intent is fewer dependent loads, since leaves sit next to their parent, and cheaper decoding, at the cost of extra device memory, a longer host build and a second traversal code path.

```diff
diff --git a/include/rt_mi355x.h b/include/rt_mi355x.h
--- a/include/rt_mi355x.h
+++ b/include/rt_mi355x.h
@@ -82,6 +82,7 @@
 #define RT_SCENE_UPDATABLE 1u
 int rt_scene_create_ex(const rt_scene_desc* desc, int device, int bvh_kind, uint32_t flags, rt_scene** out);
 #define RT_SCENE_KEEP_PREVIOUS 2u
+#define RT_SCENE_NO_COMPACT 8u
 
 typedef struct rt_scene_update_desc {
     uint32_t n_instances;
@@ -108,6 +109,8 @@
 int rt_scene_info(const rt_scene* scene, rt_scene_info_t* out);
 
 int rt_scene_check_bvh(const rt_scene* scene);
+int rt_scene_compact_bytes(const rt_scene* scene, uint64_t* out);
+int rt_scene_compact_copy(const rt_scene* scene, void* out, uint64_t capacity);
 int rt_scene_count_visits(const rt_scene* scene, uint32_t n, const float* org, const float* dir, int mode,
                           uint64_t* node_visits, uint64_t* tri_tests, float* t, uint32_t* tri);
 
@@ -198,6 +201,7 @@
     RT_K_FILL_BLACK = 11,
     RT_K_WF_SHOOT = 12,
     RT_K_BLOCK_RESOLVE = 13,
+    RT_K_COMPACT_TREE = 14,
     RT_K_COUNT = 16
 };
 
diff --git a/sycl-ray-tracer_amd/csrc/rt_abi.hip b/sycl-ray-tracer_amd/csrc/rt_abi.hip
--- a/sycl-ray-tracer_amd/csrc/rt_abi.hip
+++ b/sycl-ray-tracer_amd/csrc/rt_abi.hip
@@ -57,7 +57,7 @@
 int rt_scene_create_ex(const rt_scene_desc* desc, int device, int bvh_kind, uint32_t flags, rt_scene** out) {
     if (!out) return fail(RT_ERR_INVALID, "null output pointer");
     *out = nullptr;
-    if (flags & ~(RT_SCENE_UPDATABLE | RT_SCENE_KEEP_PREVIOUS)) return fail(RT_ERR_INVALID, "unknown scene flags");
+    if (flags & ~(RT_SCENE_UPDATABLE | RT_SCENE_KEEP_PREVIOUS | RT_SCENE_NO_COMPACT)) return fail(RT_ERR_INVALID, "unknown scene flags");
     if ((flags & RT_SCENE_KEEP_PREVIOUS) && !(flags & RT_SCENE_UPDATABLE)) return fail(RT_ERR_INVALID, "RT_SCENE_KEEP_PREVIOUS is a flag of updatable scenes: pass RT_SCENE_UPDATABLE with it");
     if (bvh_kind != RT_BVH_DEFAULT && bvh_kind != RT_BVH_LBVH && bvh_kind != RT_BVH_SAH && bvh_kind != RT_BVH_LBVH_GPU)
         return fail(RT_ERR_INVALID, "unknown bvh_kind");
@@ -84,6 +84,13 @@
         return fail(rc, err);
     }
     s->device = device;
+    if (!(flags & (RT_SCENE_UPDATABLE | RT_SCENE_NO_COMPACT)) && s->hs.built_by != RT_BVH_LBVH_GPU) {
+        rc = no_throw([&] { (void)build_compact(s->hs); return RT_OK; });
+        if (rc != RT_OK) {
+            delete s;
+            return rc;
+        }
+    }
     if (device >= 0) {
         rc = device_ok(device);
         if (rc == RT_OK) {
@@ -102,6 +109,7 @@
             for (size_t i = 0; i < s->hs.tris.size(); ++i) std::memcpy(packed.data() + i * kTriBytes, &s->hs.tris[i], std::min<size_t>(kTriBytes, sizeof(TriRec)));
             rc = upload(packed, &s->dev.tris, s->device_bytes);
         }
+        if (rc == RT_OK && !s->hs.compact.empty()) rc = upload(s->hs.compact, &s->d_compact, s->device_bytes);
         if (rc == RT_OK) rc = upload(s->hs.shade, &s->dev.shade, s->device_bytes);
         if (rc == RT_OK) {
             std::vector<InstRec> rows(s->hs.inst);
@@ -124,6 +132,11 @@
         s->dev.lds_nm = stage ? (uint32_t)std::min<size_t>(s->hs.inst.size(), kLdsNm) : 0u;
         s->dev.lds_mats = stage ? (uint32_t)std::min<size_t>(s->hs.mats.size(), kLdsMats) : 0u;
         scene_cells(s->hs, s->dev);
+        if (s->d_compact) {
+            s->dev_compact = s->dev;
+            s->dev_compact.nodes = reinterpret_cast<const BvhNode*>(s->d_compact), s->dev_compact.tris = s->d_compact;
+            s->dev_compact.n_nodes = (uint32_t)s->hs.compact.size();
+        }
     }
     if (flags & RT_SCENE_UPDATABLE) {
         rc = no_throw([&] { return init_scene_update(s, desc, (flags & RT_SCENE_KEEP_PREVIOUS) != 0); });
@@ -142,7 +155,7 @@
         for (auto& se : s->ev_gbuffer) (void)hipEventSynchronize(se.second), (void)hipEventDestroy(se.second);
         (void)hipFree((void*)s->dev.nodes), (void)hipFree((void*)s->dev.tris), (void)hipFree((void*)s->dev.shade);
         (void)hipFree((void*)s->dev.inst), (void)hipFree((void*)s->dev.mats), (void)hipFree((void*)s->dev.tex);
-        (void)hipFree((void*)s->d_query_cursor);
+        (void)hipFree((void*)s->d_query_cursor), (void)hipFree((void*)s->d_compact);
     }
     free_scene_update(s);
     delete s;
@@ -168,7 +181,21 @@
     if (const int rc0 = sync_host_copy(s)) return rc0;
     std::string err;
     int rc = check_bvh(s->hs, err);
+    if (rc == RT_OK) rc = check_compact(s->hs, err);
     return rc == RT_OK ? RT_OK : fail(rc, err);
+}
+
+int rt_scene_compact_bytes(const rt_scene* s, uint64_t* out) {
+    if (!s || !out) return fail(RT_ERR_INVALID, "null argument");
+    *out = (uint64_t)s->hs.compact.size();
+    return RT_OK;
+}
+
+int rt_scene_compact_copy(const rt_scene* s, void* out, uint64_t capacity) {
+    if (!s || !out) return fail(RT_ERR_INVALID, "null argument");
+    if (capacity < (uint64_t)s->hs.compact.size()) return fail(RT_ERR_INVALID, "buffer smaller than rt_scene_compact_bytes");
+    if (!s->hs.compact.empty()) std::memcpy(out, s->hs.compact.data(), s->hs.compact.size());
+    return RT_OK;
 }
 
 int rt_scene_count_visits(const rt_scene* s, uint32_t n, const float* org, const float* dir, int mode, uint64_t* node_visits, uint64_t* tri_tests,
diff --git a/sycl-ray-tracer_amd/csrc/rt_device.h b/sycl-ray-tracer_amd/csrc/rt_device.h
--- a/sycl-ray-tracer_amd/csrc/rt_device.h
+++ b/sycl-ray-tracer_amd/csrc/rt_device.h
@@ -298,7 +298,6 @@
     RT_CHILD(k1, ub1)
     RT_CHILD(k2, ub2)
     RT_CHILD(k3, ub3)
-#undef RT_CHILD
 #define RT_CE(KA, CA, KB, CB)                                                        \
     {                                                                               \
         const lmask sw = lanes(KB < KA);                                            \
@@ -311,7 +310,6 @@
     RT_CE(k0, c0, k1, c1)
     RT_CE(k2, c2, k3, c3)
     RT_CE(k0, c0, k2, c2)
-#undef RT_CE
     const bool descend = k0 < inf;
     if (lanes(!stack_shallow(stack, T, 3u)) == 0ull) {
         *lds_at(T.sp) = c3;
@@ -374,6 +372,121 @@
     const TravSigns sg = trav_signs(T);
     while (trav_step_wave(S, T, stack, top, sg)) {}
     return T.best;
+}
+
+struct TopCompact {
+    uint32_t base;
+    uint32_t limit;
+};
+#define RT_SDWA_BYTE(NAME, OP, K, A)                                                                                            \
+    RT_DEV uint32_t NAME(uint32_t a, uint32_t w) {                                                                           \
+        uint32_t d;                                                                                                          \
+        asm(OP " %0, %1, %2 dst_sel:DWORD dst_unused:UNUSED_PAD src0_sel:DWORD src1_sel:BYTE_" #K : "=v"(d) : A(a), "v"(w)); \
+        return d;                                                                                                            \
+    }
+RT_SDWA_BYTE(add_ub0, "v_add_u32_sdwa", 0, "v")
+RT_SDWA_BYTE(add_ub1, "v_add_u32_sdwa", 1, "v")
+RT_SDWA_BYTE(add_ub2, "v_add_u32_sdwa", 2, "v")
+RT_SDWA_BYTE(add_ub3, "v_add_u32_sdwa", 3, "v")
+RT_SDWA_BYTE(shl_ub0, "v_lshlrev_b32_sdwa", 0, "v")
+RT_SDWA_BYTE(shl_ub1, "v_lshlrev_b32_sdwa", 1, "v")
+RT_SDWA_BYTE(shl_ub2, "v_lshlrev_b32_sdwa", 2, "v")
+#undef RT_SDWA_BYTE
+RT_DEV void trav_inner(const SceneDev& S, Trav& T, const TravStack& stack, const TopCompact& top, const TravSigns& sg) {
+    const float inf = __builtin_huge_valf();
+    float k0, k1, k2, k3;
+    u32x4 w0, w1, w2;
+    if ((uint32_t)T.cur < top.limit) {
+        const uint32_t o = top.base + (uint32_t)T.cur;
+        w0 = *(lds_u32x4*)(size_t)o, w1 = *(lds_u32x4*)(size_t)(o + 16u), w2 = *(lds_u32x4*)(size_t)(o + 32u);
+    } else {
+        asm volatile("global_load_dwordx4 %0, %3, %4\n\t"
+                     "global_load_dwordx4 %1, %3, %4 offset:16\n\t"
+                     "global_load_dwordx4 %2, %3, %4 offset:32"
+                     : "=&v"(w0), "=&v"(w1), "=&v"(w2)
+                     : "v"((uint32_t)T.cur), "s"(S.nodes)
+                     : "memory");
+    }
+    asm volatile("s_waitcnt vmcnt(1)" : "+v"(w0), "+v"(w1));
+    const uint32_t sh = 23u;
+    const float ax = __uint_as_float(shl_ub0(sh, w0.w)) * T.ix;
+    const float ay = __uint_as_float(shl_ub1(sh, w0.w)) * T.iy;
+    const float az = __uint_as_float(shl_ub2(sh, w0.w)) * T.iz;
+    const float bx = __builtin_fmaf(__uint_as_float(w0.x), T.ix, T.ox);
+    const float by = __builtin_fmaf(__uint_as_float(w0.y), T.iy, T.oy);
+    const float bz = __builtin_fmaf(__uint_as_float(w0.z), T.iz, T.oz);
+    const lmask nx = sg.nx, ny = sg.ny, nz = sg.nz;
+    const uint32_t qnx = sel(nx, w1.x, w1.y), qfx = sel(nx, w1.y, w1.x);
+    const uint32_t qny = sel(ny, w1.z, w1.w), qfy = sel(ny, w1.w, w1.z);
+    asm volatile("s_waitcnt vmcnt(0)" : "+v"(w2));
+    const uint32_t qnz = sel(nz, w2.x, w2.y), qfz = sel(nz, w2.y, w2.x);
+    RT_CHILD(k0, ub0)
+    RT_CHILD(k1, ub1)
+    RT_CHILD(k2, ub2)
+    RT_CHILD(k3, ub3)
+    int32_t c0 = (int32_t)add_ub0(w2.z, w2.w), c1 = (int32_t)add_ub1(w2.z, w2.w), c2 = (int32_t)add_ub2(w2.z, w2.w), c3 = (int32_t)add_ub3(w2.z, w2.w);
+    RT_CE(k0, c0, k1, c1)
+    RT_CE(k2, c2, k3, c3)
+    RT_CE(k0, c0, k2, c2)
+    const bool descend = k0 < inf;
+    if (lanes(!stack_shallow(stack, T, 3u)) == 0ull) {
+        *lds_at(T.sp) = c3;
+        T.sp = sel(lanes(k3 < inf), T.sp, T.sp + stack.pitch);
+        *lds_at(T.sp) = c2;
+        T.sp = sel(lanes(k2 < inf), T.sp, T.sp + stack.pitch);
+        *lds_at(T.sp) = c1;
+        T.sp = sel(lanes(k1 < inf), T.sp, T.sp + stack.pitch);
+        if (descend) T.cur = c0;
+        else trav_pop_lds(T, stack);
+    } else {
+        if (k3 < inf) stk_push(stack, T, c3);
+        if (k2 < inf) stk_push(stack, T, c2);
+        if (k1 < inf) stk_push(stack, T, c1);
+        if (descend) T.cur = c0;
+        else trav_pop(T, stack);
+    }
+}
+#undef RT_CHILD
+#undef RT_CE
+RT_DEV void trav_leaf_compact(const SceneDev& S, Trav& T, const TravStack& stack) {
+    const uint8_t* p4 = S.tris + ((uint32_t)T.cur & ~3u);
+    const float4 l0 = tri_ld4(p4), l1 = tri_ld4(p4 + 16), l2 = tri_ld4(p4 + 32), l3 = tri_ld4(p4 + 48), l4 = tri_ld4(p4 + 64);
+    const bool two = ((uint32_t)T.cur & 2u) != 0u;
+    tri_test_regs(l0, l1, make_float2(l2.x, l2.y), T.o, T.d, T.best);
+    if (__ballot(two) != 0ull) {
+        if (two) tri_test_regs(make_float4(l2.z, l2.w, l3.x, l3.y), make_float4(l3.z, l3.w, l4.x, l4.y), make_float2(l4.z, l4.w), T.o, T.d, T.best);
+    }
+    if (lanes(!stack_shallow(stack, T, 0u)) == 0ull) trav_pop_lds(T, stack);
+    else trav_pop(T, stack);
+}
+RT_DEV uint32_t trav_step_wave_compact(const SceneDev& S, Trav& T, const TravStack& stack, const TopCompact& top, const TravSigns& sg) {
+    const uint32_t kind = (uint32_t)T.cur & 3u;
+    const bool inner = kind == 0u;
+    const bool leaf = !inner && T.cur != kTravDoneCompact;
+    const uint32_t ni = (uint32_t)__popcll(__ballot(inner)), nl = (uint32_t)__popcll(__ballot(leaf));
+    if (ni * 3u >= nl * 4u && !(nl >= 64u)) {
+        if (inner) trav_inner(S, T, stack, top, sg);
+    } else {
+        if (leaf) trav_leaf_compact(S, T, stack);
+    }
+    return ni + nl;
+}
+template <bool COMPACT> struct TravMode {
+    typedef TopTree Top;
+    static constexpr int32_t done = kTravDone;
+};
+template <> struct TravMode<true> {
+    typedef TopCompact Top;
+    static constexpr int32_t done = kTravDoneCompact;
+};
+template <bool STATS, bool LEAF_BATCH>
+RT_DEV uint32_t trav_step_mode(const SceneDev& S, Trav& T, const TravStack& stack, const TopTree& top, const TravSigns& sg, WaveStats* ws) {
+    return trav_step_wave<STATS, LEAF_BATCH>(S, T, stack, top, sg, ws);
+}
+template <bool STATS, bool LEAF_BATCH>
+RT_DEV uint32_t trav_step_mode(const SceneDev& S, Trav& T, const TravStack& stack, const TopCompact& top, const TravSigns& sg, WaveStats*) {
+    static_assert(!STATS && LEAF_BATCH, "the compact mode belongs to the product's one-launch kernels");
+    return trav_step_wave_compact(S, T, stack, top, sg);
 }
 
 RT_DEV bool near_zero3(f3 e) {
@@ -609,6 +722,27 @@
     const TravStack stack{(uint32_t)(size_t)(lds_i32*)(lds_stack + threadIdx.x), spill, 4u * (BLOCK)}; \
     lds_stack[threadIdx.x] = kTravDone;
 
+template <bool COMPACT> RT_DEV typename TravMode<COMPACT>::Top top_stage(const SceneDev& S, u32x4* top_all) {
+    if constexpr (COMPACT) {
+        const uint32_t bytes = S.n_nodes < kTopBytes ? S.n_nodes : kTopBytes;
+        const u32x4* in = reinterpret_cast<const u32x4*>(S.nodes);
+        for (uint32_t i = threadIdx.x; i < bytes / 16u; i += blockDim.x) top_all[i] = in[i];
+        return TopCompact{(uint32_t)(size_t)(lds_u32x4*)top_all, bytes - (uint32_t)sizeof(CompactNode) + 1u};
+    } else {
+        const int32_t top_count = (int32_t)S.n_nodes < kTopNodes ? (int32_t)S.n_nodes : kTopNodes;
+        top_tree_fill(S, top_all, top_all + kTopNodes, top_all + 2 * kTopNodes, top_all + 3 * kTopNodes, top_count);
+        return TopTree{(lds_u32x4*)top_all, (lds_u32x4*)(top_all + kTopNodes), (lds_u32x4*)(top_all + 2 * kTopNodes), (lds_u32x4*)(top_all + 3 * kTopNodes), top_count};
+    }
+}
+#define RT_TRAVERSAL_LDS_MODE(BLOCK, COMPACT)                                                          \
+    __shared__ u32x4 top_all[4 * kTopNodes];                                                           \
+    __shared__ int32_t lds_stack[kLdsStack * (BLOCK)];                                                 \
+    int32_t spill[kStackSize - kLdsStack];                                                             \
+    const typename TravMode<COMPACT>::Top top = top_stage<COMPACT>(S, top_all);                        \
+    __syncthreads();                                                                                   \
+    const TravStack stack{(uint32_t)(size_t)(lds_i32*)(lds_stack + threadIdx.x), spill, 4u * (BLOCK)}; \
+    lds_stack[threadIdx.x] = TravMode<COMPACT>::done;
+
 #define RT_SHADE_LDS                                                                                   \
     __shared__ u32x4 shade_nm[3 * kLdsNm], shade_mat[2 * kLdsMats];                                    \
     shade_tables_fill(S, shade_nm, shade_mat);                                                         \
diff --git a/sycl-ray-tracer_amd/csrc/rt_frame.hip b/sycl-ray-tracer_amd/csrc/rt_frame.hip
--- a/sycl-ray-tracer_amd/csrc/rt_frame.hip
+++ b/sycl-ray-tracer_amd/csrc/rt_frame.hip
@@ -387,7 +387,9 @@
     if (sliced) return blocks ? k_wf_finish<ST, false, false, true, true, true> : carry ? k_wf_finish<ST, false, false, true, true> : k_wf_finish<ST, false, false, true>;
     return req ? k_wf_finish<ST, true> : k_wf_finish<ST, false>;
 }
-FinishKernel finish_kernel(bool stats, bool shoot, bool req, bool sliced, bool carry, bool blocks) {
+bool finish_compact(const rt_scene* sc, bool stats, bool shoot, bool req, bool carry, bool blocks) { return sc->d_compact && !stats && !shoot && !req && !carry && !blocks; }
+FinishKernel finish_kernel(bool stats, bool shoot, bool req, bool sliced, bool carry, bool blocks, bool compact = false) {
+    if (compact) return sliced ? k_wf_finish<false, false, false, true, false, false, true> : k_wf_finish<false, false, false, false, false, false, true>;
     return stats ? finish_variant<true>(shoot, req, sliced, carry, blocks) : finish_variant<false>(shoot, req, sliced, carry, blocks);
 }
 using MegaKernel = decltype(&k_megakernel<0, false>);
@@ -402,7 +404,9 @@
 }
 template <int ST>
 MegaKernel mega_sliced(bool sliced, CarryMode carry) { return sliced ? mega_carry<ST, true>(carry) : mega_carry<ST, false>(carry); }
-MegaKernel mega_kernel(int stats, bool sliced, CarryMode carry) {
+bool mega_compact(const rt_scene* sc, int stats, CarryMode carry) { return sc->d_compact && stats == 0 && carry == kCarryNone; }
+MegaKernel mega_kernel(int stats, bool sliced, CarryMode carry, bool compact = false) {
+    if (compact) return sliced ? k_megakernel<0, true, kCarryNone, true> : k_megakernel<0, false, kCarryNone, true>;
     return stats == 2 ? mega_sliced<2>(sliced, carry) : stats == 1 ? mega_sliced<1>(sliced, carry) : mega_sliced<0>(sliced, carry);
 }
 using ShadeKernel = decltype(&k_wf_shade<false, false>);
@@ -616,8 +620,9 @@
                     if (int rc_ = fill_bytes(L.d_rq_entries, 0xFF, (size_t)L.n_local * (n_samples - 1u) * 8, ls, capturing)) return rc_;
                     if (int rc_ = fill_bytes(L.d_rq_ctl, 0, 80 * 4, ls, capturing)) return rc_;
                 }
-                const FinishKernel finish = finish_kernel(r->d_stats != nullptr, false, req, p.sl.n_slices > 1u, p.req.carry >= kCarryLoadStore, blocks);
-                hipLaunchKernelGGL(finish, dim3(fg.grid), dim3(kMegaBlock), 0, ls, S, r->d_cam, L.tile, L.q[buf[k]], counts + D0, cursors + (size_t)s * D + D0,
+                const bool compact = finish_compact(r->scene, r->d_stats != nullptr, false, req, p.req.carry >= kCarryLoadStore, blocks);
+                const FinishKernel finish = finish_kernel(r->d_stats != nullptr, false, req, p.sl.n_slices > 1u, p.req.carry >= kCarryLoadStore, blocks, compact);
+                hipLaunchKernelGGL(finish, dim3(fg.grid), dim3(kMegaBlock), 0, ls, compact ? r->scene->dev_compact : S, r->d_cam, L.tile, L.q[buf[k]], counts + D0, cursors + (size_t)s * D + D0,
                                    L.d_rng, L.d_accum, extra, D0, D, n_samples, r->rr_start, r->d_stats, fq, fg.chunk_slots,
                                    p.lpt && s == 0 ? L.d_cost : (uint8_t*)nullptr, QueueDev{}, (uint32_t*)nullptr, 0u, p.shoot_frame ? 1u : 0u, r->d_frame,
                                    p.sl.n_slices);
@@ -628,6 +633,7 @@
                 }
                 launches.add(RT_K_WF_FINISH);
                 if (req) launches.also(RT_K_WF_FINISH_REQUEUE);
+                if (compact) launches.also(RT_K_COMPACT_TREE);
             }
         }
         s += n_samples;
@@ -698,12 +704,14 @@
                 HIPCHK(hipMemsetAsync(r->d_stats + 13, 0xff, 2 * sizeof(unsigned long long), st));
                 HIPCHK(hipMemsetAsync(r->d_stats + 15, 0, 9 * sizeof(unsigned long long), st));
             }
-            const MegaKernel mega = mega_kernel(r->d_stats ? r->stats_level : 0, p.sl.n_slices > 1u, p.req.carry);
+            const bool compact = mega_compact(r->scene, r->d_stats ? r->stats_level : 0, p.req.carry);
+            const MegaKernel mega = mega_kernel(r->d_stats ? r->stats_level : 0, p.sl.n_slices > 1u, p.req.carry, compact);
             const uint32_t pad = r->mega_lds_pad;
             if (pad) (void)hipFuncSetAttribute((const void*)mega, hipFuncAttributeMaxDynamicSharedMemorySize, (int)pad);
-            hipLaunchKernelGGL(mega, dim3(p.grid), dim3(kMegaBlock), pad, st, S, r->d_frame, c.width, c.height, r->tile, r->max_depth, p.req.spp, r->seed_mode,
+            hipLaunchKernelGGL(mega, dim3(p.grid), dim3(kMegaBlock), pad, st, compact ? r->scene->dev_compact : S, r->d_frame, c.width, c.height, r->tile, r->max_depth, p.req.spp, r->seed_mode,
                                r->rr_start, d_f32, d_u8, r->d_ray_counter, r->d_stats, p.sl.n_slices);
             launches.add(p.hot);
+            if (compact) launches.also(RT_K_COMPACT_TREE);
         }
         HIPCHK(hipGetLastError());
         HIPCHK(hipEventRecord(e1, st));
diff --git a/sycl-ray-tracer_amd/csrc/rt_internal.h b/sycl-ray-tracer_amd/csrc/rt_internal.h
--- a/sycl-ray-tracer_amd/csrc/rt_internal.h
+++ b/sycl-ray-tracer_amd/csrc/rt_internal.h
@@ -116,6 +116,8 @@
     HostScene hs;
     int device = -1;
     SceneDev dev{};
+    const uint8_t* d_compact = nullptr;
+    SceneDev dev_compact{};
     uint64_t device_bytes = 0;
     SceneUpdate* upd = nullptr;
     uint64_t generation = 0;
diff --git a/sycl-ray-tracer_amd/csrc/rt_kernels.h b/sycl-ray-tracer_amd/csrc/rt_kernels.h
--- a/sycl-ray-tracer_amd/csrc/rt_kernels.h
+++ b/sycl-ray-tracer_amd/csrc/rt_kernels.h
@@ -176,12 +176,14 @@
     const uint32_t base = (uint32_t)(size_t)planes;
     return (lds_u32_word*)(size_t)(base + 3u * kMegaBlock * 4u + (((a - base) >> 6) & ~3u));
 }
-template <int STATS, bool SLICED, int CARRY = 0>
+template <int STATS, bool SLICED, int CARRY = 0, bool COMPACT = false>
 __global__ void __launch_bounds__(kMegaBlock, kMegaWaves) k_megakernel(SceneDev S, const MegaFrame* frame, int32_t width, int32_t height, TileDev tile,
                                                     uint32_t max_depth, uint32_t spp, uint32_t seed_mode, uint32_t rr_start, float* __restrict__ out_f32,
                                                     uint8_t* __restrict__ out_u8,
                                                     unsigned long long* __restrict__ ray_counter,
                                                     unsigned long long* __restrict__ stats_out, uint32_t n_slices) {
+    static_assert(!COMPACT || (STATS == 0 && CARRY == 0), "the compact traversal buffer is the product's: no statistics, no carried state");
+    constexpr int32_t kDone = TravMode<COMPACT>::done;
     WaveStats ws;
     long long t_begin = 0, t_mark = 0, t_trav = 0, t_shade = 0;
     long long ck[8] = {0, 0, 0, 0, 0, 0, 0, 0};
@@ -205,8 +207,8 @@
     Trav T;
     if (SLICED) *slice_looks_word(color_r, (lds_f32*)color_lds) = 0u;
     RT_SHADE_LDS
-    RT_TRAVERSAL_LDS(kMegaBlock)
-    T.cur = kTravDone;
+    RT_TRAVERSAL_LDS_MODE(kMegaBlock, COMPACT)
+    T.cur = kDone;
     constexpr uint32_t kPend = 0x40000000u;
     bool live = false;
     RefillPolicy refill;
@@ -292,21 +294,21 @@
         const uint32_t n_rays = SLICED ? (uint32_t)__popcll(__ballot(live && depth < kPend)) : n_live;
         const uint32_t shade_at = n_rays * kMegaShadePct + (n_live - n_rays) * 100u;
         for (;;) {
-            const bool waiting = live && T.cur == kTravDone;
+            const bool waiting = live && T.cur == kDone;
             if ((uint32_t)__popcll(__ballot(waiting)) * 100u >= shade_at) break;
             if (STATS >= 2) ws.live_lane_steps += n_live;
             if (STATS == 1) ws.inner_steps += (uint32_t)kMegaUnroll;
             refill.stepped();
-            (void)trav_step_wave<(STATS >= 2), true>(S, T, stack, top, sg, &ws);
+            (void)trav_step_mode<(STATS >= 2), true>(S, T, stack, top, sg, &ws);
 #pragma unroll
             for (int k = 1; k < kMegaUnroll; ++k) {
                 if (STATS >= 2) ws.live_lane_steps += n_live;
-                (void)trav_step_wave<(STATS >= 2), true>(S, T, stack, top, sg, &ws);
+                (void)trav_step_mode<(STATS >= 2), true>(S, T, stack, top, sg, &ws);
             }
         }
         if (STATS) {
             ws.shade_rounds++;
-            if (STATS >= 2) ws.shade_lanes += (uint32_t)__popcll(__ballot(live && T.cur == kTravDone));
+            if (STATS >= 2) ws.shade_lanes += (uint32_t)__popcll(__ballot(live && T.cur == kDone));
             const long long now = (long long)__builtin_readcyclecounter();
             t_trav += now - t_mark, t_mark = now;
         }
@@ -316,11 +318,11 @@
 #endif
         bool pixel_finished = false;
         {
-            const unsigned long long traced = __ballot(live && T.cur == kTravDone && depth < kPend);
+            const unsigned long long traced = __ballot(live && T.cur == kDone && depth < kPend);
             wave_rays += (unsigned long long)__popcll(traced);
             if (SLICED && traced == 0ull && __ballot(live && depth < kPend) == 0ull && slice_wait_count(slice_looks_word(color_r, (lds_f32*)color_lds), frame) && lane == 0) atomicMax(ray_counter + 2, 1ull);
         }
-        if (live && T.cur == kTravDone) {
+        if (live && T.cur == kDone) {
             bool start = false;
             if (SLICED && depth >= kPend) {
                 const SliceNow sn = frame_slices(frame);
@@ -689,7 +691,7 @@
 RT_DEV unsigned long long rq_load64(const unsigned long long* p) { return __hip_atomic_load(p, __ATOMIC_RELAXED, __HIP_MEMORY_SCOPE_AGENT); }
 RT_DEV void rq_store64(unsigned long long* p, unsigned long long v) { __hip_atomic_store(p, v, __ATOMIC_RELAXED, __HIP_MEMORY_SCOPE_AGENT); }
 
-template <bool STATS, bool REQ, bool LIMIT = false, bool SLICED = false, bool CARRY = false, bool BLOCKS = false>
+template <bool STATS, bool REQ, bool LIMIT = false, bool SLICED = false, bool CARRY = false, bool BLOCKS = false, bool COMPACT = false>
 __global__ void __launch_bounds__(kMegaBlock, kMegaWaves) k_wf_finish(SceneDev S, const CameraDev* __restrict__ camp, TileDev tile, QueueDev qin,
                                                                     const uint32_t* __restrict__ count_in, uint32_t* __restrict__ cursor,
                                                                     uint32_t* __restrict__ rng_buf, float4* __restrict__ accum,
@@ -702,6 +704,8 @@
     static_assert(!(SLICED && (REQ || LIMIT)), "pixel slices belong to the one-launch schedule");
     static_assert(!CARRY || SLICED, "only the sliced schedule keeps a pixel's sums outside the accumulator");
     static_assert(!BLOCKS || CARRY, "a block continuation is a continuation");
+    static_assert(!COMPACT || !(STATS || REQ || LIMIT || CARRY), "the compact traversal buffer is the one-launch product's: unsliced or sliced, nothing else");
+    constexpr int32_t kDone = TravMode<COMPACT>::done;
     constexpr uint32_t kPend = 0x40000000u;
     const bool holes = (qflags & 1u) != 0u;
     __shared__ unsigned long long out_word;
@@ -716,7 +720,7 @@
     const uint32_t wave_id = blockIdx.x * kWavesPerBlock + (threadIdx.x >> 6);
     const uint32_t n_waves = gridDim.x * kWavesPerBlock;
     RT_SHADE_LDS
-    RT_TRAVERSAL_LDS(kMegaBlock)
+    RT_TRAVERSAL_LDS_MODE(kMegaBlock, COMPACT)
     __shared__ unsigned long long rq_stage_mem[REQ ? kWavesPerBlock * kRqStage : 1u];
     typedef __attribute__((address_space(3))) unsigned long long lds_u64_t;
     lds_u64_t* stage = (lds_u64_t*)rq_stage_mem + (threadIdx.x >> 6) * kRqStage;
@@ -742,7 +746,7 @@
     bool drained = false;
     bool waiting = false;
     Trav T;
-    T.cur = kTravDone;
+    T.cur = kDone;
     bool live = false;
     RefillPolicy refill;
     RayState r{};
@@ -926,24 +930,24 @@
         const uint32_t n_rays = SLICED ? (uint32_t)__popcll(__ballot(live && depth < kPend)) : n_live;
         const uint32_t shade_at = n_rays * kMegaShadePct + (n_live - n_rays) * 100u;
         for (;;) {
-            const bool done_trav = live && T.cur == kTravDone;
+            const bool done_trav = live && T.cur == kDone;
             if ((uint32_t)__popcll(__ballot(done_trav)) * 100u >= shade_at) break;
             if (STATS) ws.live_lane_steps += n_live * kMegaUnroll;
             refill.stepped();
-            (void)trav_step_wave<STATS, true>(S, T, stack, top, sg, &ws);
+            (void)trav_step_mode<STATS, true>(S, T, stack, top, sg, &ws);
 #pragma unroll
-            for (int k = 1; k < kMegaUnroll; ++k) (void)trav_step_wave<STATS, true>(S, T, stack, top, sg, &ws);
-        }
-        if (STATS) ws.shade_rounds++, ws.shade_lanes += (uint32_t)__popcll(__ballot(live && T.cur == kTravDone));
+            for (int k = 1; k < kMegaUnroll; ++k) (void)trav_step_mode<STATS, true>(S, T, stack, top, sg, &ws);
+        }
+        if (STATS) ws.shade_rounds++, ws.shade_lanes += (uint32_t)__popcll(__ballot(live && T.cur == kDone));
         __builtin_amdgcn_s_setprio(0);
         bool requeue = false, slot_finished = false, hand_on = false;
         {
-            const unsigned long long traced = __ballot(live && T.cur == kTravDone && !(SLICED && depth >= kPend));
-            wave_rays += (unsigned long long)__popcll(__ballot(live && T.cur == kTravDone && !(first_counted && depth == first_depth) && !(SLICED && depth >= kPend)));
+            const unsigned long long traced = __ballot(live && T.cur == kDone && !(SLICED && depth >= kPend));
+            wave_rays += (unsigned long long)__popcll(__ballot(live && T.cur == kDone && !(first_counted && depth == first_depth) && !(SLICED && depth >= kPend)));
             if (SLICED && traced == 0ull && __ballot(live && depth < kPend) == 0ull && slice_wait_count(slice_looks_word(sum_r, (lds_f32_t*)sum_lds), slices) && lane == 0 && fq.error)
                 __hip_atomic_store(fq.error, 4u, __ATOMIC_RELAXED, __HIP_MEMORY_SCOPE_AGENT);
         }
-        if (SLICED && live && T.cur == kTravDone && depth >= kPend) {
+        if (SLICED && live && T.cur == kDone && depth >= kPend) {
             const SliceNow sn = frame_slices(slices);
             const auto rsrc = state_rsrc(sn);
             const uint32_t at = id * 32u, tag = sn.head.z + (n_samples - samples_left);
@@ -964,7 +968,7 @@
                 depth = 0;
                 trav_begin(T, r.org, ray_dir(r), stack);
             }
-        } else if (live && T.cur == kTravDone) {
+        } else if (live && T.cur == kDone) {
             f3 res;
             const bool done = shade_bounce<true>(S, rng, r, T.best, res, &T, &tab);
             depth++;
diff --git a/sycl-ray-tracer_amd/csrc/rt_types.h b/sycl-ray-tracer_amd/csrc/rt_types.h
--- a/sycl-ray-tracer_amd/csrc/rt_types.h
+++ b/sycl-ray-tracer_amd/csrc/rt_types.h
@@ -51,9 +51,30 @@
 
 constexpr int kMaxLeafTris = 2;
 constexpr int kTopNodes = 341;
+constexpr uint32_t kTopBytes = (uint32_t)kTopNodes * 64u;
 constexpr int kStackSize = 64;
 constexpr uint32_t kNoTri = 0xFFFFFFFFu;
 constexpr float kTNear = 0.0001f;
+
+struct alignas(16) CompactNode {
+    float origin[3];
+    uint32_t exps;
+    uint32_t q[6];
+    uint32_t base;
+    uint32_t f;
+};
+static_assert(sizeof(CompactNode) == 48, "CompactNode must be 48 bytes");
+constexpr uint32_t kCompactTail = 48;
+constexpr uint32_t kCompactMaxDelta = 252;
+constexpr uint32_t kCompactKindLeaf1 = 1, kCompactKindLeaf2 = 2;
+constexpr int32_t kTravDoneCompact = -1;
+RT_HD uint32_t compact_child(const CompactNode& n, int k) { return n.base + ((n.f >> (8 * k)) & 0xffu); }
+RT_HD uint32_t compact_exps(const BvhNode& n) {
+    const float s[3] = {n.scale(0), n.scale(1), n.scale(2)};
+    uint32_t w = 0;
+    for (int a = 0; a < 3; ++a) w |= ((__builtin_bit_cast(uint32_t, s[a]) >> 23) & 0xffu) << (8 * a);
+    return w;
+}
 
 struct ContractRange {
     float lo[3], hi[3];
diff --git a/sycl-ray-tracer_amd/csrc/scene_build.cpp b/sycl-ray-tracer_amd/csrc/scene_build.cpp
--- a/sycl-ray-tracer_amd/csrc/scene_build.cpp
+++ b/sycl-ray-tracer_amd/csrc/scene_build.cpp
@@ -781,6 +781,60 @@
     }
 }
 
+bool build_compact(HostScene& hs) {
+    hs.compact.clear(), hs.compact_at.clear();
+    if (hs.nodes.empty() || hs.max_leaf_tris > 2u) return false;
+    if ((uint64_t)hs.nodes.size() * 64u + (uint64_t)hs.tris.size() * kTriBytes + 128u > 0xFFFFFF00ull) return false;
+    std::vector<uint8_t>& out = hs.compact;
+    hs.compact_at.assign(hs.nodes.size(), 0u);
+    out.assign(sizeof(CompactNode), 0);
+    struct Item { int32_t node; float area; };
+    std::deque<Item> q{{0, 0.0f}};
+    while (!q.empty()) {
+        Item it;
+        if (out.size() < (size_t)kTopBytes) {
+            size_t pick = 0;
+            for (size_t i = 1; i < q.size(); ++i)
+                if (q[i].area > q[pick].area) pick = i;
+            it = q[pick];
+            q.erase(q.begin() + (std::ptrdiff_t)pick);
+        } else { it = q.back(); q.pop_back(); }
+        const BvhNode& n = hs.nodes[(size_t)it.node];
+        CompactNode c;
+        std::memcpy(c.origin, n.origin, 12);
+        c.exps = compact_exps(n);
+        std::memcpy(c.q, n.q, 24);
+        const size_t base = (out.size() + 15u) & ~(size_t)15u;
+        size_t at = base;
+        c.base = (uint32_t)base, c.f = 0u;
+        Item pending[4];
+        int n_pending = 0;
+        for (int k = 0; k < 4; ++k) {
+            if (n.child[k] < 0) continue;
+            c.f |= (uint32_t)(at - base) << (8 * k);
+            hs.compact_at[(size_t)n.child[k]] = (uint32_t)at;
+            const Box3 b = child_box(n, k);
+            pending[n_pending++] = {n.child[k], half_area(b.lo, b.hi)};
+            at += sizeof(CompactNode);
+        }
+        out.resize(at, 0);
+        for (int k = 0; k < 4; ++k) {
+            if (n.child[k] >= 0 || n.child[k] == kChildEmpty) continue;
+            const LeafRange leaf = leaf_range(n.child[k]);
+            c.f |= ((uint32_t)(out.size() - base) | leaf.count) << (8 * k);
+            for (uint32_t j = 0; j < leaf.count; ++j) {
+                const uint8_t* rec = reinterpret_cast<const uint8_t*>(&hs.tris[(size_t)leaf.first + j]);
+                out.insert(out.end(), rec, rec + kTriBytes);
+            }
+        }
+        std::memcpy(out.data() + hs.compact_at[(size_t)it.node], &c, sizeof c);
+        if (out.size() < (size_t)kTopBytes) for (int k = 0; k < n_pending; ++k) q.push_back(pending[k]);
+        else for (int k = n_pending - 1; k >= 0; --k) q.push_back(pending[k]);
+    }
+    out.resize(((out.size() + 15u) & ~(size_t)15u) + kCompactTail, 0);
+    return true;
+}
+
 void world_vertices(uint32_t n_tris, const uint32_t* indices, const uint32_t* tri_instance, const rt_instance* inst, const float* positions,
                     std::vector<float>& wv) {
     wv.resize(9 * (size_t)n_tris);
diff --git a/sycl-ray-tracer_amd/csrc/scene_build.h b/sycl-ray-tracer_amd/csrc/scene_build.h
--- a/sycl-ray-tracer_amd/csrc/scene_build.h
+++ b/sycl-ray-tracer_amd/csrc/scene_build.h
@@ -26,6 +26,8 @@
     float pad = 0.0f;
     uint32_t max_depth = 0, max_leaf_tris = 0, stack_need = 0;
     double sah_cost = 0.0;
+    std::vector<uint8_t> compact;
+    std::vector<uint32_t> compact_at;
 };
 
 constexpr int RT_BVH_MEDIAN_INTERNAL = 99;
@@ -54,7 +56,10 @@
 double refit_sah_cost(const HostScene& hs, const std::vector<float>& box);
 double decoded_sah_cost(const HostScene& hs);
 
+bool build_compact(HostScene& hs);
+
 int check_bvh(const HostScene& hs, std::string& err);
+int check_compact(const HostScene& hs, std::string& err);
 
 int count_visits(const HostScene& hs, uint32_t n, const float* org, const float* dir, int mode, uint64_t* node_visits, uint64_t* tri_tests, float* t_out,
                  uint32_t* tri_out, std::string& err);
diff --git a/sycl-ray-tracer_amd/csrc/scene_check.cpp b/sycl-ray-tracer_amd/csrc/scene_check.cpp
--- a/sycl-ray-tracer_amd/csrc/scene_check.cpp
+++ b/sycl-ray-tracer_amd/csrc/scene_check.cpp
@@ -2,6 +2,7 @@
 
 #include <algorithm>
 #include <cmath>
+#include <cstring>
 #include <limits>
 
 namespace rt {
@@ -132,10 +133,137 @@
     return RT_OK;
 }
 
+int check_compact(const HostScene& hs, std::string& err) {
+    if (hs.compact.empty()) return RT_OK;
+    const std::vector<uint8_t>& buf = hs.compact;
+    const size_t size = buf.size();
+    auto fail = [&](const std::string& m, int32_t node) { err = "compact buffer: " + m + " (node " + std::to_string(node) + ")"; return RT_ERR_INVALID; };
+    if (hs.nodes.empty() || size < sizeof(CompactNode) + kCompactTail || size % 16u) return fail("bad size", 0);
+    std::vector<std::pair<int32_t, uint32_t>> todo{{0, 0u}};
+    size_t visited = 0;
+    while (!todo.empty()) {
+        const int32_t cn = todo.back().first;
+        const uint32_t off = todo.back().second;
+        todo.pop_back();
+        if (cn < 0 || (size_t)cn >= hs.nodes.size() || ++visited > hs.nodes.size()) return fail("node graph does not match the canonical tree's", cn);
+        if (off % 16u) return fail("node not 16-byte aligned", cn);
+        if ((size_t)off + sizeof(CompactNode) + kCompactTail > size) return fail("node outside the buffer", cn);
+        CompactNode c;
+        std::memcpy(&c, buf.data() + off, sizeof c);
+        const BvhNode& n = hs.nodes[(size_t)cn];
+        if (std::memcmp(c.origin, n.origin, 12) != 0) return fail("origin differs", cn);
+        if (c.exps != compact_exps(n)) return fail("grid-step exponents differ", cn);
+        if (std::memcmp(c.q, n.q, 24) != 0) return fail("plane words differ", cn);
+        if (c.base % 16u) return fail("group not 16-byte aligned", cn);
+        size_t expect = c.base;
+        for (int pass = 0; pass < 2; ++pass)
+            for (int k = 0; k < 4; ++k) {
+                const uint32_t byte = (c.f >> (8 * k)) & 0xffu, kind = byte & 3u, delta = byte & ~3u;
+                const int32_t child = n.child[k];
+                if (child == kChildEmpty) {
+                    if (pass == 0 && byte != 0u) return fail("absent child with a child byte", cn);
+                    continue;
+                }
+                if ((child >= 0) != (pass == 0)) continue;
+                if (delta > kCompactMaxDelta || delta % 8u) return fail("bad delta", cn);
+                if (c.base < off + sizeof(CompactNode)) return fail("group not behind its parent", cn);
+                if ((size_t)c.base + delta != expect) return fail("group not contiguous", cn);
+                if (child >= 0) {
+                    if (kind != 0u) return fail("inner child with a leaf kind", cn);
+                    if (compact_child(c, k) != expect) return fail("child word differs", cn);
+                    todo.emplace_back(child, (uint32_t)expect);
+                    expect += sizeof(CompactNode);
+                } else {
+                    const LeafRange leaf = leaf_range(child);
+                    if (kind != leaf.count || leaf.count > 2u) return fail("leaf record count differs", cn);
+                    if ((size_t)leaf.first + leaf.count > hs.tris.size()) return fail("canonical leaf out of range", cn);
+                    if (expect + 2u * kTriBytes > size) return fail("the 80-byte leaf read leaves the buffer", cn);
+                    for (uint32_t j = 0; j < leaf.count; ++j)
+                        if (std::memcmp(buf.data() + expect + (size_t)j * kTriBytes, &hs.tris[(size_t)leaf.first + j], kTriBytes) != 0) return fail("leaf record bytes differ", cn);
+                    expect += (size_t)leaf.count * kTriBytes;
+                }
+            }
+        if (expect + kCompactTail > size) return fail("group outside the buffer", cn);
+    }
+    if (visited != hs.nodes.size()) return fail("fewer nodes than the canonical tree", 0);
+    return RT_OK;
+}
+
+static int count_visits_compact(const HostScene& hs, uint32_t n, const float* org, const float* dir, uint64_t* node_visits, uint64_t* tri_tests, float* t_out,
+                                uint32_t* tri_out) {
+    const float inf = std::numeric_limits<float>::infinity();
+    const uint8_t* buf = hs.compact.data();
+    uint64_t visits = 0, tests = 0;
+    for (uint32_t i = 0; i < n; ++i) {
+        const float o[3] = {org[3 * i], org[3 * i + 1], org[3 * i + 2]}, d[3] = {dir[3 * i], dir[3 * i + 1], dir[3 * i + 2]};
+        float inv[3];
+        for (int a = 0; a < 3; ++a) inv[a] = 1.0f / (std::fabs(d[a]) < 1e-30f ? std::copysign(1e-30f, d[a]) : d[a]);
+        float best = inf;
+        uint32_t best_tri = kNoTri;
+        uint32_t stack[kStackSize * 4];
+        int sp = 0;
+        uint32_t cur = 0;
+        for (;;) {
+            if ((cur & 3u) == 0u) {
+                visits++;
+                CompactNode nd;
+                std::memcpy(&nd, buf + cur, sizeof nd);
+                float key[4];
+                uint32_t ch[4];
+                int m = 0;
+                for (int k = 0; k < 4; ++k) {
+                    float tn = 0.0f, tf = best;
+                    bool absent = true;
+                    for (int a = 0; a < 3; ++a) {
+                        const float step = __builtin_bit_cast(float, ((nd.exps >> (8 * a)) & 0xffu) << 23);
+                        const uint32_t ql = (nd.q[2 * a] >> (8 * k)) & 0xffu, qh = (nd.q[2 * a + 1] >> (8 * k)) & 0xffu;
+                        absent = absent && ql == 255u && qh == 0u;
+                        const float lo = nd.origin[a] + (float)ql * step, hi = nd.origin[a] + (float)qh * step;
+                        const float t0 = (lo - o[a]) * inv[a], t1 = (hi - o[a]) * inv[a];
+                        tn = std::max(tn, std::min(t0, t1)), tf = std::min(tf, std::max(t0, t1));
+                    }
+                    if (absent && ((nd.f >> (8 * k)) & 0xffu) == 0u) continue;
+                    if (tn <= tf) key[m] = tn, ch[m] = compact_child(nd, k), m++;
+                }
+                for (int a = 1; a < m; ++a)
+                    for (int b = a; b > 0 && key[b] < key[b - 1]; --b) std::swap(key[b], key[b - 1]), std::swap(ch[b], ch[b - 1]);
+                for (int a = m - 1; a >= 1; --a) stack[sp++] = ch[a];
+                if (m) { cur = ch[0]; continue; }
+            } else {
+                const uint32_t count = cur & 3u;
+                for (uint32_t k = 0; k < count; ++k) {
+                    tests++;
+                    TriRec tr{};
+                    std::memcpy(&tr, buf + (cur & ~3u) + k * kTriBytes, kTriBytes);
+                    const double e1[3] = {tr.e1[0], tr.e1[1], tr.e1[2]}, e2[3] = {tr.e2[0], tr.e2[1], tr.e2[2]};
+                    const double p[3] = {d[1] * e2[2] - d[2] * e2[1], d[2] * e2[0] - d[0] * e2[2], d[0] * e2[1] - d[1] * e2[0]};
+                    const double det = e1[0] * p[0] + e1[1] * p[1] + e1[2] * p[2];
+                    if (det == 0.0) continue;
+                    const double tv[3] = {o[0] - tr.v0[0], o[1] - tr.v0[1], o[2] - tr.v0[2]};
+                    const double u = (tv[0] * p[0] + tv[1] * p[1] + tv[2] * p[2]) / det;
+                    const double q[3] = {tv[1] * e1[2] - tv[2] * e1[1], tv[2] * e1[0] - tv[0] * e1[2], tv[0] * e1[1] - tv[1] * e1[0]};
+                    const double v = (d[0] * q[0] + d[1] * q[1] + d[2] * q[2]) / det;
+                    if (u < 0.0 || v < 0.0 || u + v > 1.0) continue;
+                    const double t = (e2[0] * q[0] + e2[1] * q[1] + e2[2] * q[2]) / det;
+                    if (t > (double)kTNear && (t < best || (t == best && tr.global_index < best_tri))) best = (float)t, best_tri = tr.global_index;
+                }
+            }
+            if (sp == 0) break;
+            cur = stack[--sp];
+        }
+        if (t_out) t_out[i] = best;
+        if (tri_out) tri_out[i] = best_tri;
+    }
+    if (node_visits) *node_visits = visits;
+    if (tri_tests) *tri_tests = tests;
+    return RT_OK;
+}
+
 int count_visits(const HostScene& hs, uint32_t n, const float* org, const float* dir, int mode, uint64_t* node_visits, uint64_t* tri_tests, float* t_out,
                  uint32_t* tri_out, std::string& err) {
     if (mode < 0 || mode > 2) { err = "mode: 0 quantised, 1 exact, 2 quantised with two more bits"; return RT_ERR_INVALID; }
     if (hs.nodes.empty()) { err = "no tree"; return RT_ERR_INVALID; }
+    if (mode == 0 && !hs.compact.empty()) return count_visits_compact(hs, n, org, dir, node_visits, tri_tests, t_out, tri_out);
     const float inf = std::numeric_limits<float>::infinity();
     std::vector<Box3> box(hs.nodes.size() * 4);
     auto tested = [&](int32_t node, int k, const Box3& c) {
diff --git a/sycl-ray-tracer_amd/rtamd/abi.py b/sycl-ray-tracer_amd/rtamd/abi.py
--- a/sycl-ray-tracer_amd/rtamd/abi.py
+++ b/sycl-ray-tracer_amd/rtamd/abi.py
@@ -19,6 +19,7 @@
 RT_BVH_MEDIAN_INTERNAL = 99
 RT_SCENE_UPDATABLE = 1
 RT_SCENE_KEEP_PREVIOUS = 2
+RT_SCENE_NO_COMPACT = 8
 RT_TEX_SIZE = 512
 RT_TEX_MAX_LAYERS = 128
 
@@ -109,7 +110,7 @@
 RT_SCHED_ALL_BOUNCES = 0xFFFFFFFF
 KERNELS = {"megakernel": 0, "wf_init": 1, "wf_generate": 2, "wf_extend": 3, "wf_shade": 4, "wf_shade_reorder": 5, "wf_shade_matsort": 6,
            "wf_finish": 7, "wf_finish_requeue": 8, "wf_tile_order": 9, "wf_resolve": 10, "fill_black": 11, "wf_shoot": 12,
-           "block_resolve": 13}
+           "block_resolve": 13, "compact_tree": 14}
 RT_K_COUNT = 16
 
 
@@ -230,6 +231,8 @@
     "rt_scene_update": (C.c_int, [C.c_void_p, _P(rt_scene_update_desc), _P(rt_update_stats)]),
     "rt_scene_info": (C.c_int, [C.c_void_p, _P(rt_scene_info_t)]),
     "rt_scene_check_bvh": (C.c_int, [C.c_void_p]),
+    "rt_scene_compact_bytes": (C.c_int, [C.c_void_p, _P(C.c_uint64)]),
+    "rt_scene_compact_copy": (C.c_int, [C.c_void_p, C.c_void_p, C.c_uint64]),
     "rt_scene_count_visits": (C.c_int, [C.c_void_p, C.c_uint32, _P(C.c_float), _P(C.c_float), C.c_int, _P(C.c_uint64), _P(C.c_uint64),
                                          _P(C.c_float), _P(C.c_uint32)]),
     "rt_intersect_batch": (C.c_int, [C.c_void_p, C.c_uint32, _P(C.c_float), _P(C.c_float), _P(C.c_float),
diff --git a/sycl-ray-tracer_amd/rtamd/renderer.py b/sycl-ray-tracer_amd/rtamd/renderer.py
--- a/sycl-ray-tracer_amd/rtamd/renderer.py
+++ b/sycl-ray-tracer_amd/rtamd/renderer.py
@@ -27,14 +27,14 @@
 class Scene:
 
     def __init__(self, desc: SceneDesc, device: int = 0, bvh: int = abi.RT_BVH_DEFAULT, lib=None, updatable: bool = False,
-                 keep_previous: bool = False):
+                 keep_previous: bool = False, no_compact: bool = False):
         self.desc = desc
         self.device = device
         self._lib = lib or abi.load_library()
         self._c = desc.to_c()
         self.h = C.c_void_p()
-        if updatable or keep_previous:
-            flags = (abi.RT_SCENE_UPDATABLE if updatable else 0) | (abi.RT_SCENE_KEEP_PREVIOUS if keep_previous else 0)
+        if updatable or keep_previous or no_compact:
+            flags = (abi.RT_SCENE_UPDATABLE if updatable else 0) | (abi.RT_SCENE_KEEP_PREVIOUS if keep_previous else 0) | (abi.RT_SCENE_NO_COMPACT if no_compact else 0)
             abi.check(self._lib.rt_scene_create_ex(C.byref(self._c), device, bvh, flags, C.byref(self.h)), self._lib)
         else:
             abi.check(self._lib.rt_scene_create(C.byref(self._c), device, bvh, C.byref(self.h)), self._lib)
@@ -70,6 +70,11 @@
         abi.check(self._lib.rt_scene_info(self.h, C.byref(out)), self._lib)
         return out
 
+    def compact_bytes(self) -> int:
+        out = C.c_uint64()
+        abi.check(self._lib.rt_scene_compact_bytes(self.h, C.byref(out)), self._lib)
+        return int(out.value)
+
     def check_bvh(self) -> None:
         abi.check(self._lib.rt_scene_check_bvh(self.h), self._lib)
 
```

Measured after the change: 9269. 0.943x the previous value.
